# orybkin/video-gcp

Measured on AMD Instinct MI355X. Metric: predicted frames/sec, 64x64x3 seq_len=80 gcp_tree (posterior forward + all loss terms, model(inputs) and model.loss() of train.py:157-159, batch-stat BatchNorm), higher is better.
Workload: dtype f32 (encoder / decoder convs and the tree GEMMs from 512 rows: split-f16 MFMA with f32 accumulate, f32-equivalent; everything else exact f32 MFMA)

## Files before the change

### video-gcp_amd/csrc/gemm.hip

```cpp
#include "common.h"
#include "gemm_tile.h"

#include <cstdio>
#include <cstdlib>
#include <type_traits>

bool gcpx_gemm_split_applies(const gcpx_gemm_args* a);
int gcpx_launch_gemm_split(const gcpx_gemm_args* a, hipStream_t stream);
bool gcpx_gemm_planes_applies(const gcpx_gemm_args* a);
int gcpx_launch_gemm_planes(const gcpx_gemm_args* a, hipStream_t stream);

namespace {

template <int PR, int CR, bool LSTM, bool KS = false>
__global__ void __launch_bounds__(256) gemm_kernel(const gcpx_gemm_args a) {
    gemm_tile<PR, CR, LSTM, KS>(a, blockIdx.x, blockIdx.y, blockIdx.z);
}

__global__ void __launch_bounds__(256) gemm_group_kernel(const gcpx_gemm_args* __restrict__ tab, const int4* __restrict__ dims, const int n) {
    int p = 0;
    while (p + 1 < n && (int)blockIdx.x >= dims[p + 1].x) ++p;
    const int4 d = dims[p];
    const int local = blockIdx.x - d.x;
    const int bx = local % d.y, by = (local / d.y) % d.z, bz = local / (d.y * d.z);
    const gcpx_gemm_args& a = tab[p];
    if (a.epi == GCPX_EPI_GAUSS_SAMPLE) {
        const int r = bx * 16 + ((int)threadIdx.x >> 4), d = by * 16 + ((int)threadIdx.x & 15);
        if (r < a.M) {
            const int b = r / a.rpb, j = r % a.rpb;
            const float* m = a.src[0].ptr + (size_t)b * a.src[0].sb + (size_t)j * a.src[0].sr;
            const float e = a.src[1].ptr[(size_t)b * a.src[1].sb + (size_t)j * a.src[1].sr + d];
            a.out[(size_t)b * a.ob + (size_t)j * a.orow + d] = m[d] + expf(m[a.N + d]) * e;
        }
        return;
    }
    if (a.epi == GCPX_EPI_LSTM) gemm_tile<1, 1, true, true>(a, bx, by, bz);
    else gemm_tile<1, 1, false, true>(a, bx, by, bz);
}

struct TileChoice { int pr, cr; };

TileChoice choose_tile(int M, int N, int nb = 1) {
    if (const char* ov = getenv("GCPX_GEMM_TILE")) {
        int pr = 0, cr = 0, mm = 0;
        if (sscanf(ov, "%d,%d,%d", &pr, &cr, &mm) == 3 && M >= mm && N % (16 * cr) == 0) return TileChoice{pr, cr};
    }
    static const long simds = [] {
        int dev = 0, cus = 256;
        if (hipGetDevice(&dev) == hipSuccess) (void)hipDeviceGetAttribute(&cus, hipDeviceAttributeMultiprocessorCount, dev);
        return 4L * (cus > 0 ? cus : 256);
    }();
    const int prs[3] = {4, 2, 1}, crs[3] = {4, 2, 1};
    TileChoice best{1, 1};
    double best_cost = -1.0, best_bytes = 0.0;
    const long NT = N / 16, RT = (M + 15) / 16;
    if (M >= 64 && N % 64 == 0 && ((RT + 3) / 4) * (NT / 4) * nb >= simds) return TileChoice{4, 4};
    for (int pi = 0; pi < 3; ++pi)
        for (int ci = 0; ci < 3; ++ci) {
            const int pr = prs[pi], cr = crs[ci];
            if (N % (16 * cr)) continue;
            if (pr > 1 && 16 * pr > ((M + 15) & ~15)) continue;
            const long waves = ((RT + pr - 1) / pr) * ((NT + cr - 1) / cr) * nb;
            const long rounds = (waves + simds - 1) / simds;
            const int area = pr * cr;
            const double e = area >= 16 ? 4.2 : area >= 8 ? 4.9 : area >= 4 ? 5.0 : area >= 2 ? 6.0 : 8.0;
            const double compute = (double)rounds * area * e * (rounds > 1 ? 1.35 : 1.0);
            const double bytes = 256.0 * (pr + cr) / area;
            const double l2 = (double)RT * NT * nb * 256.0 * bytes / 1.0e7;
            const double cost = compute > l2 ? compute : l2;
            if (best_cost < 0 || cost < best_cost - 1e-9 || (cost < best_cost + 1e-9 && bytes < best_bytes)) {
                best_cost = cost; best_bytes = bytes; best = TileChoice{pr, cr};
            }
        }
    return best;
}

template <int PR, int CR>
void launch_t(const gcpx_gemm_args* a, hipStream_t stream) {
    const int rbk = (a->M + 16 * PR - 1) / (16 * PR);
    const int cbk = (a->N / 16 + 4 * CR - 1) / (4 * CR);
    const int nb = a->nbatch > 1 ? a->nbatch : 1;
    if (a->epi == GCPX_EPI_LSTM)
        hipLaunchKernelGGL((gemm_kernel<PR, CR, true>), dim3(rbk, cbk, nb), dim3(256), 0, stream, *a);
    else
        hipLaunchKernelGGL((gemm_kernel<PR, CR, false>), dim3(rbk, cbk, nb), dim3(256), 0, stream, *a);
}

}

extern "C" int gcpx_gemm_row_blocks(int32_t M, int32_t N) {
    const TileChoice t = choose_tile(M, N);
    return (M + 16 * t.pr - 1) / (16 * t.pr);
}

static int gemm_check(const gcpx_gemm_args* a);

static bool ks_block_choice(const gcpx_gemm_args* a, int* pr_out, int* cr_out) {
    static const int max_rows = [] { const char* e = getenv("GCPX_GEMM_KS_MAX_ROWS"); return e ? atoi(e) : 4096; }();
    static const int max_cost = [] { const char* e = getenv("GCPX_GEMM_KS_MAX_COST"); return e ? atoi(e) : 6; }();
    if (!(a->M >= 64 && a->M <= max_rows && a->K >= 256 && !a->stats_partial) || getenv("GCPX_GEMM_NO_KS_BLOCKS")) return false;
    static const long cus = [] {
        int dev = 0, n = 256;
        if (hipGetDevice(&dev) == hipSuccess) (void)hipDeviceGetAttribute(&n, hipDeviceAttributeMultiprocessorCount, dev);
        return (long)(n > 0 ? n : 256);
    }();
    const long nb = a->nbatch > 1 ? a->nbatch : 1;
    const int shapes[5][2] = {{1, 1}, {1, 2}, {2, 2}, {4, 2}, {2, 4}};
    int best = 0;
    long best_cost = -1;
    for (int i = 0; i < 5; ++i) {
        const int pr = shapes[i][0], cr = shapes[i][1];
        if (a->N % (16 * cr)) continue;
        const long wgs = (long)((a->M + 16 * pr - 1) / (16 * pr)) * (a->N / (16 * cr)) * nb;
        const long cost = ((wgs + cus - 1) / cus) * (pr + cr);
        if (best_cost < 0 || cost < best_cost) { best_cost = cost; best = i; }
    }
    if (best == 0 || best_cost > max_cost) return false;
    *pr_out = shapes[best][0];
    *cr_out = shapes[best][1];
    return true;
}

static bool gemm_is_small(const gcpx_gemm_args* a) {
    int pr_ = 1, cr_ = 1;
    if (ks_block_choice(a, &pr_, &cr_)) return false;
    const int nb = a->nbatch > 1 ? a->nbatch : 1;
    const TileChoice t = choose_tile(a->M, a->N, nb);
    const long rbk = (a->M + 15) / 16, nt = a->N / 16;
    return t.pr == 1 && t.cr == 1 && a->K >= 256 && rbk * nt * nb <= 1024 && !a->stats_partial;
}

extern "C" int gcpx_gemm_group_dims(const gcpx_gemm_args* host_table, int32_t n, int32_t* dims, int32_t* total_blocks) {
    GCPX_CHECK_ARG(host_table && dims && total_blocks && n >= 1 && n <= 16, "bad arguments");
    int start = 0;
    for (int p = 0; p < n; ++p) {
        if (host_table[p].epi == GCPX_EPI_GAUSS_SAMPLE) {
            const gcpx_gemm_args& a = host_table[p];
            GCPX_CHECK_ARG(a.nsrc == 2 && a.src[0].ptr && a.src[1].ptr && a.out && a.M > 0 && a.N > 0 && a.N % 16 == 0 && a.rpb > 0 &&
                               a.src[0].width == 2 * a.N && a.src[1].width == a.N, "gauss sample: [mu | log_sigma] rows, eps rows, out");
            dims[4 * p] = start; dims[4 * p + 1] = (a.M + 15) / 16; dims[4 * p + 2] = a.N / 16; dims[4 * p + 3] = 1;
            start += dims[4 * p + 1] * dims[4 * p + 2];
            continue;
        }
        const int st = gemm_check(host_table + p);
        if (st != GCPX_OK) return st;
        if (!gemm_is_small(host_table + p)) {
            gcpx_set_error("gcpx_gemm_group_dims: problem %d (M=%d N=%d K=%d) is not in the small-M split-K regime", p, host_table[p].M,
                           host_table[p].N, host_table[p].K);
            return GCPX_ERR_UNSUPPORTED;
        }
        const int nb = host_table[p].nbatch > 1 ? host_table[p].nbatch : 1;
        const int rbk = (host_table[p].M + 15) / 16, nt = host_table[p].N / 16;
        dims[4 * p] = start; dims[4 * p + 1] = rbk; dims[4 * p + 2] = nt; dims[4 * p + 3] = nb;
        start += rbk * nt * nb;
    }
    *total_blocks = start;
    return GCPX_OK;
}

extern "C" int gcpx_gemm_group(const gcpx_gemm_args* dev_table, const int32_t* dev_dims, int32_t n, int32_t total_blocks, void* stream_) {
    hipStream_t stream = reinterpret_cast<hipStream_t>(stream_);
    GCPX_CHECK_ARG(dev_table && dev_dims && n >= 1 && n <= 16 && total_blocks > 0, "bad arguments");
    GCPX_CHECK_ARG((((uintptr_t)dev_dims) & 15) == 0, "dims must be 16-byte aligned");
    hipLaunchKernelGGL(gemm_group_kernel, dim3(total_blocks), dim3(256), 0, stream, dev_table, reinterpret_cast<const int4*>(dev_dims), n);
    GCPX_CHECK_LAUNCH();
    return GCPX_OK;
}

static int gemm_check(const gcpx_gemm_args* a) {
    GCPX_CHECK_ARG(a != nullptr, "null args");
    GCPX_CHECK_ARG(a->epi != GCPX_EPI_GAUSS_SAMPLE, "GCPX_EPI_GAUSS_SAMPLE is a gcpx_gemm_group problem");
    GCPX_CHECK_ARG(a->nsrc >= 1 && a->nsrc <= 6, "nsrc out of range");
    GCPX_CHECK_ARG(a->M > 0 && a->N > 0 && a->N % 16 == 0 && a->rpb > 0, "bad M/N/rpb");
    int ksum = 0;
    for (int s = 0; s < a->nsrc; ++s) {
        GCPX_CHECK_ARG(a->src[s].ptr != nullptr, "source pointer is NULL");
        GCPX_CHECK_ARG(a->src[s].width > 0 && a->src[s].width % 16 == 0, "source width must be a multiple of 16");
        GCPX_CHECK_ARG(!(a->src[s].scale || a->src[s].act) ||
                           (a->src[s].cmod > 0 && (a->src[s].cmod & (a->src[s].cmod - 1)) == 0),
                       "cmod must be a power of two when scale/act is set");
        ksum += a->src[s].width;
    }
    GCPX_CHECK_ARG(ksum == a->K, "K != sum of source widths");
    GCPX_CHECK_ARG(a->wpk != nullptr, "weights missing");
    if (a->epi == GCPX_EPI_LSTM) {
        GCPX_CHECK_ARG(a->c_prev && a->h_out && a->c_out, "LSTM epilogue needs c_prev/h_out/c_out");
    } else {
        GCPX_CHECK_ARG(a->out != nullptr, "out is NULL");
    }
    GCPX_CHECK_ARG(a->nbatch <= 1 || (a->epi != GCPX_EPI_LSTM && !a->stats_partial), "nbatch > 1 only for plain epilogues");
    GCPX_CHECK_ARG(!a->lstm_bwd || (a->epi == GCPX_EPI_NONE && a->nbatch <= 1 && !a->stats_partial),
                   "lstm_bwd: plain epilogue, single problem");
    return GCPX_OK;
}

bool gcpx_gemm_tile_plan(const gcpx_gemm_args* a, int* pr, int* cr, int* ks, int* gx, int* gy, int* gz) {
    if (gemm_check(a) != GCPX_OK || a->stats_partial) return false;
    const int nb = a->nbatch > 1 ? a->nbatch : 1;
    *gz = nb;
    if (ks_block_choice(a, pr, cr)) {
        *ks = 1; *gx = (a->M + 16 * *pr - 1) / (16 * *pr); *gy = a->N / (16 * *cr);
        return true;
    }
    if (gcpx_gemm_split_applies(a)) return false;
    const TileChoice t = choose_tile(a->M, a->N, nb);
    const long rbk = (a->M + 15) / 16, nt = a->N / 16;
    if (t.pr == 1 && t.cr == 1 && a->K >= 256 && !getenv("GCPX_GEMM_NOKS") && rbk * nt * nb <= 1024) {
        *pr = 1; *cr = 1; *ks = 1; *gx = (int)rbk; *gy = (int)nt;
        return true;
    }
    *pr = t.pr; *cr = t.cr; *ks = 0;
    *gx = (a->M + 16 * t.pr - 1) / (16 * t.pr); *gy = (a->N / 16 + 4 * t.cr - 1) / (4 * t.cr);
    return true;
}

extern "C" int gcpx_gemm(const gcpx_gemm_args* a, void* stream_) {
    hipStream_t stream = reinterpret_cast<hipStream_t>(stream_);
    const int st = gemm_check(a);
    if (st != GCPX_OK) return st;
    {
        int pr_ = 1, cr_ = 1;
        if (!ks_block_choice(a, &pr_, &cr_)) {
            if (gcpx_gemm_planes_applies(a)) return gcpx_launch_gemm_planes(a, stream);
            if (gcpx_gemm_split_applies(a)) return gcpx_launch_gemm_split(a, stream);
        }
    }
    const TileChoice t = choose_tile(a->M, a->N, a->nbatch > 1 ? a->nbatch : 1);
    {
        int pr = 1, cr = 1;
        if (ks_block_choice(a, &pr, &cr)) {
            const long nb = a->nbatch > 1 ? a->nbatch : 1;
            const dim3 grid((a->M + 16 * pr - 1) / (16 * pr), a->N / (16 * cr), nb);
            const bool lstm = a->epi == GCPX_EPI_LSTM;
#define GCPX_KS_LAUNCH(PR_, CR_)                                                                                              \
            do {                                                                                                              \
                if (lstm) hipLaunchKernelGGL((gemm_kernel<PR_, CR_, true, true>), grid, dim3(256), 0, stream, *a);            \
                else hipLaunchKernelGGL((gemm_kernel<PR_, CR_, false, true>), grid, dim3(256), 0, stream, *a);                \
            } while (0)
            if (pr == 1 && cr == 2) GCPX_KS_LAUNCH(1, 2);
            else if (pr == 2 && cr == 2) GCPX_KS_LAUNCH(2, 2);
            else if (pr == 4 && cr == 2) GCPX_KS_LAUNCH(4, 2);
            else GCPX_KS_LAUNCH(2, 4);
#undef GCPX_KS_LAUNCH
            GCPX_CHECK_LAUNCH();
            return GCPX_OK;
        }
    }
    if (t.pr == 1 && t.cr == 1 && a->K >= 256 && !getenv("GCPX_GEMM_NOKS")) {
        const long nb = a->nbatch > 1 ? a->nbatch : 1;
        const long rbk = (a->M + 15) / 16, nt = a->N / 16;
        if (rbk * nt * nb <= 1024) {
            if (a->epi == GCPX_EPI_LSTM)
                hipLaunchKernelGGL((gemm_kernel<1, 1, true, true>), dim3(rbk, nt, nb), dim3(256), 0, stream, *a);
            else
                hipLaunchKernelGGL((gemm_kernel<1, 1, false, true>), dim3(rbk, nt, nb), dim3(256), 0, stream, *a);
            GCPX_CHECK_LAUNCH();
            return GCPX_OK;
        }
    }
    switch (t.pr * 10 + t.cr) {
        case 44: launch_t<4, 4>(a, stream); break;
        case 42: launch_t<4, 2>(a, stream); break;
        case 41: launch_t<4, 1>(a, stream); break;
        case 24: launch_t<2, 4>(a, stream); break;
        case 22: launch_t<2, 2>(a, stream); break;
        case 21: launch_t<2, 1>(a, stream); break;
        case 14: launch_t<1, 4>(a, stream); break;
        case 12: launch_t<1, 2>(a, stream); break;
        default: launch_t<1, 1>(a, stream); break;
    }
    GCPX_CHECK_LAUNCH();
    return GCPX_OK;
}
```

### video-gcp_amd/csrc/gemm_split.hip

```cpp
#include "common.h"

#include <cstdlib>
#include <type_traits>

namespace {

typedef _Float16 h8 __attribute__((ext_vector_type(8)));
typedef _Float16 h4 __attribute__((ext_vector_type(4)));
typedef const f32x4 __attribute__((address_space(1)))* gptr4;
__device__ __forceinline__ float4 gload4(const float* p) {
    const f32x4 t = *(gptr4)p;
    return make_float4(t[0], t[1], t[2], t[3]);
}

__device__ __forceinline__ f32x4 mfma32h(h8 a, h8 b, f32x4 c) {
    return __builtin_amdgcn_mfma_f32_16x16x32_f16(a, b, c, 0, 0, 0);
}

template <int TN, int NSUB, int NW = 4>
struct GsCfg {
    static constexpr int TM = 16 * NW, THREADS = 64 * NW, KS = 32 * NSUB;
    static constexpr int NCT = TN / 16;
    static constexpr int W_SUB = NCT * 2048;
    static constexpr int W_BYTES = NSUB * W_SUB;
    static constexpr int X_SUB = NW * 2048;
    static constexpr int X_BYTES = NSUB * X_SUB;
    static constexpr int STAGE = W_BYTES + X_BYTES + 4 * TM;
    static constexpr int LDS_BYTES = 2 * STAGE;
    static constexpr int WLD = W_BYTES / (THREADS * 16);
    static constexpr int WSTEP = THREADS * 16;
};

template <int TN, int NSUB, bool LSTM, bool XF, int NW = 4>
__global__ void __launch_bounds__(64 * NW) gemm_split_kernel(const gcpx_gemm_args a) {
    using Cfg = GsCfg<TN, NSUB, NW>;
    constexpr int KS = Cfg::KS;
    constexpr int NCT = Cfg::NCT, WLD = Cfg::WLD, CPW = NCT / 2;
    extern __shared__ float4 smem4[];
    char* smem = reinterpret_cast<char*>(smem4);
    const int tid = threadIdx.x, lane = tid & 63, wave = tid >> 6;
    const int j = lane & 15, q = lane >> 4;
    const int wr = wave >> 1, wc = wave & 1;
    const int zb = blockIdx.z;
    const int NT = a.N / 16;
    const int ct0 = blockIdx.y * NCT;
    const int M = a.M, rpb = a.rpb;
    const int NK = a.K / KS;

    const int srow = (wave << 4) + j, kq = q;
    const int sr_ = blockIdx.x * Cfg::TM + srow;
    const bool srv = sr_ < M;
    const int srs = srv ? sr_ : 0;
    const int srb = srs / rpb, srj = srs % rpb;
    const int ew = a.w_split_log2_dev ? a.w_split_log2_dev[zb] : a.w_split_log2;
    const int ex_cap = min(100, 126 - ew);
    int ex_run = ex_cap;
    int cur_s = -1, krem = 0, kloc = 0;
    const float* xp = nullptr;
    float xmask = 0.f;
    const float* sp[6];
    float sm[6];
    int sw[6];
#pragma unroll
    for (int i = 0; i < 6; ++i) {
        sp[i] = a.src[0].ptr; sm[i] = 0.f; sw[i] = 0;
        if (i < a.nsrc) {
            sw[i] = a.src[i].width / KS;
            const gcpx_row_src& src = a.src[i];
            bool ok = srv;
            size_t off;
            if (src.rowidx) {
                off = (size_t)src.rowidx[srs] * src.sr;
            } else {
                const int jj = srj + src.shift;
                ok = ok && jj >= 0 && jj < rpb;
                off = (size_t)srb * src.sb + (size_t)(ok ? jj : 0) * src.sr;
            }
            sp[i] = src.ptr + (size_t)zb * a.z_src_off + off + kq * 8;
            sm[i] = ok ? 1.f : 0.f;
        }
    }
    auto next_source = [&]() {
        ++cur_s;
        xp = sp[0]; xmask = sm[0]; krem = sw[0];
#pragma unroll
        for (int i = 1; i < 6; ++i)
            if (cur_s == i) { xp = sp[i]; xmask = sm[i]; krem = sw[i]; }
        kloc = 0;
    };
    const char* wsrc = reinterpret_cast<const char*>(a.wpk_split) + (size_t)zb * a.z_w_off * 4 + (size_t)ct0 * 2048 + tid * 16;

    struct RegSet {
        float4 x[2 * NSUB], w[WLD];
        float mask;
        int src, k0;
    };
    RegSet rs[2];
    const float* last_x = sp[0];
    int last_s = 0;
    auto issue = [&](const int s, RegSet& r) __attribute__((always_inline)) {
        if (s < NK) {
            if (krem == 0) next_source();
            last_x = xp + kloc;
            last_s = s;
            r.mask = xmask; r.src = cur_s; r.k0 = kloc;
            kloc += KS;
            --krem;
        }
#pragma unroll
        for (int h = 0; h < NSUB; ++h) {
            r.x[2 * h] = gload4(last_x + 32 * h);
            r.x[2 * h + 1] = gload4(last_x + 32 * h + 4);
        }
#pragma unroll
        for (int i = 0; i < WLD; ++i) {
            const int sub = i / (WLD / NSUB), c = i % (WLD / NSUB);
            r.w[i] = *reinterpret_cast<const float4*>(wsrc + ((size_t)(NSUB * last_s + sub) * NT) * 2048 + c * Cfg::WSTEP);
        }
    };
    auto commit = [&](const int st, RegSet& r) __attribute__((always_inline)) {
        char* base = smem + st * Cfg::STAGE;
#pragma unroll
        for (int i = 0; i < WLD; ++i) {
            const int sub = i / (WLD / NSUB), c = i % (WLD / NSUB);
            *reinterpret_cast<float4*>(base + sub * Cfg::W_SUB + c * Cfg::WSTEP + tid * 16) = r.w[i];
        }
        if constexpr (XF) {
#pragma unroll
            for (int si = 0; si < 6; ++si) {
                if (r.src == si && (a.src[si].scale || a.src[si].act)) {
#pragma unroll
                    for (int i = 0; i < 2 * NSUB; ++i)
                        r.x[i] = affine_act4(r.x[i], a.src[si].scale, a.src[si].shiftv,
                                             (r.k0 + 32 * (i >> 1) + 4 * (i & 1) + kq * 8) & (a.src[si].cmod - 1), a.src[si].act);
                }
            }
        }
        float amax = 0.f;
#pragma unroll
        for (int i = 0; i < 2 * NSUB; ++i) {
            float4 v = r.x[i];
            v.x *= r.mask; v.y *= r.mask; v.z *= r.mask; v.w *= r.mask;
            r.x[i] = v;
            amax = fmaxf(amax, fmaxf(fmaxf(fabsf(v.x), fabsf(v.y)), fmaxf(fabsf(v.z), fabsf(v.w))));
        }
        {
            unsigned u = __float_as_uint(amax);
            auto s16 = __builtin_amdgcn_permlane16_swap(u, u, false, false);
            u = max(s16[0], s16[1]);
            auto s32 = __builtin_amdgcn_permlane32_swap(u, u, false, false);
            amax = __uint_as_float(max(s32[0], s32[1]));
        }
        if (amax > 0.f) {
            const int ec = 14 + 127 - (int)((__float_as_uint(amax) >> 23) & 0xff);
            ex_run = min(ex_run, max(-100, ec));
        }
        const float sc = __uint_as_float((unsigned)(127 + ex_run) << 23);
        char* xb = base + Cfg::W_BYTES + (wave * 2) * 1024 + lane * 16;
#pragma unroll
        for (int h = 0; h < NSUB; ++h) {
            const float4 v0 = r.x[2 * h], v1 = r.x[2 * h + 1];
            const float f[8] = {v0.x * sc, v0.y * sc, v0.z * sc, v0.w * sc, v1.x * sc, v1.y * sc, v1.z * sc, v1.w * sc};
            h8 p1, p2;
#pragma unroll
            for (int e = 0; e < 8; ++e) {
                p1[e] = (_Float16)f[e];
                p2[e] = (_Float16)fmaf((float)p1[e], -1.f, f[e]);
            }
            *reinterpret_cast<h8*>(xb + h * Cfg::X_SUB) = p1;
            *reinterpret_cast<h8*>(xb + h * Cfg::X_SUB + 1024) = p2;
        }
        if (kq == 0) *reinterpret_cast<int*>(base + Cfg::W_BYTES + Cfg::X_BYTES + srow * 4) = ex_run;
    };

    f32x4 acc[CPW][2];
#pragma unroll
    for (int c = 0; c < CPW; ++c) { acc[c][0] = f32x4{0, 0, 0, 0}; acc[c][1] = f32x4{0, 0, 0, 0}; }
    int excur[2] = {ex_cap, ex_cap};
    auto compute = [&](const int st) __attribute__((always_inline)) {
        const char* base = smem + st * Cfg::STAGE;
        int en[2];
#pragma unroll
        for (int i = 0; i < 2; ++i) en[i] = *reinterpret_cast<const int*>(base + Cfg::W_BYTES + Cfg::X_BYTES + ((2 * wr + i) * 16 + j) * 4);
        if (__any(en[0] != excur[0] || en[1] != excur[1])) {
#pragma unroll
            for (int i = 0; i < 2; ++i) {
                const int d = en[i] - excur[i];
                const float r = d < -126 ? 0.f : __uint_as_float((unsigned)(127 + d) << 23);
#pragma unroll
                for (int c = 0; c < CPW; ++c) acc[c][i] *= r;
                excur[i] = en[i];
            }
        }
#pragma unroll
        for (int sub = 0; sub < NSUB; ++sub) {
            h8 b[2][2];
#pragma unroll
            for (int i = 0; i < 2; ++i) {
                const char* bp = base + Cfg::W_BYTES + sub * Cfg::X_SUB + ((2 * wr + i) * 2) * 1024 + lane * 16;
                b[i][0] = *reinterpret_cast<const h8*>(bp);
                b[i][1] = *reinterpret_cast<const h8*>(bp + 1024);
            }
            constexpr int CH = CPW <= 4 ? CPW : 2;
#pragma unroll
            for (int c0 = 0; c0 < CPW; c0 += CH) {
                h8 w[CH][2];
#pragma unroll
                for (int c = 0; c < CH; ++c) {
                    const char* wp = base + sub * Cfg::W_SUB + ((wc * CPW + c0 + c) * 2) * 1024 + lane * 16;
                    w[c][0] = *reinterpret_cast<const h8*>(wp);
                    w[c][1] = *reinterpret_cast<const h8*>(wp + 1024);
                }
#pragma unroll
                for (int c = 0; c < CH; ++c)
#pragma unroll
                    for (int i = 0; i < 2; ++i) acc[c0 + c][i] = mfma32h(w[c][1], b[i][0], acc[c0 + c][i]);
#pragma unroll
                for (int c = 0; c < CH; ++c)
#pragma unroll
                    for (int i = 0; i < 2; ++i) acc[c0 + c][i] = mfma32h(w[c][0], b[i][1], acc[c0 + c][i]);
#pragma unroll
                for (int c = 0; c < CH; ++c)
#pragma unroll
                    for (int i = 0; i < 2; ++i) acc[c0 + c][i] = mfma32h(w[c][0], b[i][0], acc[c0 + c][i]);
            }
        }
    };

    issue(0, rs[0]);
    issue(1, rs[1]);
    commit(0, rs[0]);
    issue(2, rs[0]);
    __syncthreads();
    for (int s = 0; s < NK; s += 2) {
        compute(0);
        __builtin_amdgcn_sched_barrier(0);
        commit(1, rs[1]);
        issue(s + 3, rs[1]);
        __syncthreads();
        if (s + 1 >= NK) break;
        compute(1);
        __builtin_amdgcn_sched_barrier(0);
        commit(0, rs[0]);
        issue(s + 4, rs[0]);
        __syncthreads();
    }

#pragma unroll
    for (int i = 0; i < 2; ++i) {
        const int r = blockIdx.x * Cfg::TM + (2 * wr + i) * 16 + j;
        const bool rv = r < M;
        const int rs = rv ? r : 0;
        const int rb = rs / rpb, rj = rs % rpb;
        const float inv = __uint_as_float((unsigned)(127 - excur[i] - ew) << 23);
#pragma unroll
        for (int c = 0; c < CPW; ++c) {
            const int nt = ct0 + wc * CPW + c;
            const int n = nt * 16 + q * 4;
            float4 bv = make_float4(0.f, 0.f, 0.f, 0.f);
            if (a.bias) bv = *reinterpret_cast<const float4*>(a.bias + (size_t)zb * a.z_bias_off + n);
            f32x4 v = acc[c][i];
            v[0] = fmaf(v[0], inv, bv.x); v[1] = fmaf(v[1], inv, bv.y); v[2] = fmaf(v[2], inv, bv.z); v[3] = fmaf(v[3], inv, bv.w);
            if (!rv) continue;
            if constexpr (LSTM) {
                const int u = nt * 4 + q;
                const float cp = a.c_prev[(size_t)r * a.c_prev_stride + u];
                const float ig = sigmoidf_(v[0]), fg = sigmoidf_(v[1]), gg = tanhf(v[2]), og = sigmoidf_(v[3]);
                const float cn = fg * cp + ig * gg;
                const float h = og * tanhf(cn);
                const size_t o = (size_t)rb * a.hb + (size_t)rj * a.hrow + u;
                a.h_out[o] = h;
                a.c_out[o] = cn;
                if (a.h_copy) a.h_copy[(size_t)r * (a.N / 4) + u] = h;
                if (a.gates_out)
                    *reinterpret_cast<float4*>(a.gates_out + ((size_t)r * (a.N / 4) + u) * 4) = make_float4(ig, fg, gg, og);
            } else {
                if (a.epi == GCPX_EPI_LRELU) {
                    v[0] = lrelu(v[0], 0.2f); v[1] = lrelu(v[1], 0.2f); v[2] = lrelu(v[2], 0.2f); v[3] = lrelu(v[3], 0.2f);
                }
                float* op = a.out + (size_t)zb * a.z_out_off + (size_t)rb * a.ob + (size_t)rj * a.orow + n;
                *reinterpret_cast<float4*>(op) = make_float4(v[0], v[1], v[2], v[3]);
            }
        }
    }
}

template <int TN, int NSUB, int NW = 4>
int launch_split(const gcpx_gemm_args* a, hipStream_t stream) {
    using Cfg = GsCfg<TN, NSUB, NW>;
    static bool attr_set = false;
    if (!attr_set) {
        for (const void* k : {reinterpret_cast<const void*>(gemm_split_kernel<TN, NSUB, false, false, NW>), reinterpret_cast<const void*>(gemm_split_kernel<TN, NSUB, true, false, NW>),
                              reinterpret_cast<const void*>(gemm_split_kernel<TN, NSUB, false, true, NW>), reinterpret_cast<const void*>(gemm_split_kernel<TN, NSUB, true, true, NW>)}) {
            hipError_t e = hipFuncSetAttribute(k, hipFuncAttributeMaxDynamicSharedMemorySize, Cfg::LDS_BYTES);
            if (e != hipSuccess) {
                gcpx_set_error("gemm split: hipFuncSetAttribute(%d B LDS): %s", Cfg::LDS_BYTES, hipGetErrorString(e));
                return GCPX_ERR_HIP;
            }
        }
        attr_set = true;
    }
    const int nb = a->nbatch > 1 ? a->nbatch : 1;
    const dim3 grid((a->M + Cfg::TM - 1) / Cfg::TM, a->N / TN, nb);
    bool xf = false;
    for (int s = 0; s < a->nsrc; ++s) xf = xf || a->src[s].scale || a->src[s].act;
    const bool lstm = a->epi == GCPX_EPI_LSTM;
    auto kern = lstm ? (xf ? gemm_split_kernel<TN, NSUB, true, true, NW> : gemm_split_kernel<TN, NSUB, true, false, NW>)
                     : (xf ? gemm_split_kernel<TN, NSUB, false, true, NW> : gemm_split_kernel<TN, NSUB, false, false, NW>);
    hipLaunchKernelGGL(kern, grid, dim3(Cfg::THREADS), Cfg::LDS_BYTES, stream, *a);
    GCPX_CHECK_LAUNCH();
    return GCPX_OK;
}

}

bool gcpx_gemm_split_applies(const gcpx_gemm_args* a) {
    static const int min_rows = [] { const char* e = getenv("GCPX_GEMM_SPLIT_MIN_ROWS"); return e ? atoi(e) : 512; }();
    if (!a->wpk_split || a->M < min_rows || a->N % 64 || a->stats_partial || a->lstm_bwd) return false;
    for (int s = 0; s < a->nsrc; ++s)
        if (a->src[s].width % 64) return false;
    return true;
}

int gcpx_launch_gemm_split(const gcpx_gemm_args* a, hipStream_t stream) {
    const long nb = a->nbatch > 1 ? a->nbatch : 1;
    const long rbk = (a->M + 63) / 64;
    static const int force = [] { const char* e = getenv("GCPX_GEMM_SPLIT_CFG"); return e ? atoi(e) : 0; }();
    if (force == 1282) return launch_split<128, 2>(a, stream);
    if (force == 642) return launch_split<64, 2>(a, stream);
    if (force == 641) return launch_split<64, 1>(a, stream);
    if (force == 1281) return launch_split<128, 1>(a, stream);
    if (force == 2561 && a->N % 256 == 0) return launch_split<256, 1>(a, stream);
    if (force == 1288 && a->N % 128 == 0) return launch_split<128, 1, 8>(a, stream);
    if (force == 2568 && a->N % 256 == 0) return launch_split<256, 1, 8>(a, stream);
    if (a->N % 256 == 0 && ((a->M + 127) / 128) * (long)(a->N / 256) * nb >= 256) return launch_split<256, 1, 8>(a, stream);
    if (a->N % 128 == 0 && ((a->M + 127) / 128) * (long)(a->N / 128) * nb >= 512) return launch_split<128, 1, 8>(a, stream);
    if (a->N % 128 == 0 && rbk * (a->N / 128) * nb >= 768) return launch_split<128, 1>(a, stream);
    return launch_split<64, 1>(a, stream);
}
```

### video-gcp_amd/csrc/mlp.hip

```cpp
#include "common.h"
#include "gemm_tile.h"

#include <cstdlib>

bool gcpx_gemm_tile_plan(const gcpx_gemm_args* a, int* pr, int* cr, int* ks, int* gx, int* gy, int* gz);

namespace {

template <int MID, bool LEAN>
__device__ __forceinline__ void mlp_rows(const gcpx_mlp_args& a, const int bx, const int by, const int ny, float* hid) {
    constexpr int NTM = MID / 16;
    constexpr int NW = NTM >= 4 ? 4 : NTM;
    constexpr int TPW = NTM / NW;
    constexpr int PITCH = MID + 4;
    constexpr int CPG = MID / 8;
    static_assert(CPG == 4 || CPG == 16, "GroupNorm group must be one lane (4) or one 16-channel tile");

    const int lane = threadIdx.x & 63, wave = threadIdx.x >> 6;
    const int j = lane & 15, q = lane >> 4;
    const int r = bx * 16 + j;
    const bool rv = r < a.M;
    const int rs = rv ? r : 0;
    const int rb = rs / a.rpb, rj = rs % a.rpb;
    const float slope = a.lrelu_slope;
    const bool owner = wave < NW;
    const int nt0 = wave * TPW;

    f32x4 acc[TPW];
#pragma unroll
    for (int t = 0; t < TPW; ++t) acc[t] = f32x4{0, 0, 0, 0};

    auto load_hidden = [&](const int l, float4 (&w)[NTM][TPW]) {
        const float4* wbase = reinterpret_cast<const float4*>(a.w_mid) + ((size_t)l * NTM * NTM + nt0) * 64 + lane;
#pragma unroll
        for (int kg = 0; kg < NTM; ++kg)
#pragma unroll
            for (int t = 0; t < TPW; ++t) w[kg][t] = wbase[(kg * NTM + t) * 64];
    };
    float4 wA[NTM][TPW], wB[NTM][TPW];
    if (!LEAN && owner && a.n_mid > 0) load_hidden(0, wA);

    if (owner) {
        const float4* wbase = reinterpret_cast<const float4*>(a.w_in) + (size_t)nt0 * 64 + lane;
        int kg0 = 0;
        for (int s = 0; s < a.nsrc; ++s) {
            const gcpx_row_src src = a.src[s];
            bool ok = rv;
            size_t off;
            if (src.rowidx) {
                off = (size_t)src.rowidx[rs] * src.sr;
            } else {
                const int jj = rj + src.shift;
                ok = ok && jj >= 0 && jj < a.rpb;
                off = (size_t)rb * src.sb + (size_t)(ok ? jj : 0) * src.sr;
            }
            const float* bp = src.ptr + off + q * 4;
            const float mask = ok ? 1.f : 0.f;
            const int nkg = src.width / 16;
            const bool xf = src.scale || src.act;
            constexpr int UKI = LEAN ? 4 : 8;
            auto load_set = [&](const int kg, float4 (&b)[UKI], float4 (&w)[UKI][TPW]) {
#pragma unroll
                for (int u = 0; u < UKI; ++u) {
                    const int k = (kg + u < nkg) ? kg + u : nkg - 1;
                    b[u] = *reinterpret_cast<const float4*>(bp + k * 16);
#pragma unroll
                    for (int t = 0; t < TPW; ++t) w[u][t] = wbase[((size_t)(kg0 + k) * NTM + t) * 64];
                }
            };
            auto mfma_set = [&](const int kg, float4 (&b)[UKI], float4 (&w)[UKI][TPW]) {
#pragma unroll
                for (int u = 0; u < UKI; ++u) {
                    if (kg + u < nkg) {
                        float4 bb = b[u];
                        if (xf) bb = affine_act4(bb, src.scale, src.shiftv, ((kg + u) * 16 + q * 4) & (src.cmod - 1), src.act);
                        bb.x *= mask; bb.y *= mask; bb.z *= mask; bb.w *= mask;
#pragma unroll
                        for (int t = 0; t < TPW; ++t) {
                            acc[t] = mfma16(w[u][t].x, bb.x, acc[t]);
                            acc[t] = mfma16(w[u][t].y, bb.y, acc[t]);
                            acc[t] = mfma16(w[u][t].z, bb.z, acc[t]);
                            acc[t] = mfma16(w[u][t].w, bb.w, acc[t]);
                        }
                    }
                }
            };
            float4 b0[UKI], w0[UKI][TPW], b1[UKI], w1[UKI][TPW];
            int kg = 0;
            load_set(0, b0, w0);
            while (true) {
                const int kn = kg + UKI;
                if (kn < nkg) load_set(kn, b1, w1);
                mfma_set(kg, b0, w0);
                if (kn >= nkg) break;
                kg = kn + UKI;
                if (kg < nkg) load_set(kg, b0, w0);
                mfma_set(kn, b1, w1);
                if (kg >= nkg) break;
            }
            kg0 += nkg;
        }
#pragma unroll
        for (int t = 0; t < TPW; ++t) {
            const int c = (nt0 + t) * 16 + q * 4;
            const float4 bv = *reinterpret_cast<const float4*>(a.b_in + c);
            float4 v = make_float4(lrelu(acc[t][0] + bv.x, slope), lrelu(acc[t][1] + bv.y, slope),
                                   lrelu(acc[t][2] + bv.z, slope), lrelu(acc[t][3] + bv.w, slope));
            *reinterpret_cast<float4*>(hid + j * PITCH + c) = v;
            if (a.save && rv && by == 0) *reinterpret_cast<float4*>(a.save + (size_t)r * MID + c) = v;
        }
    }
    __syncthreads();

    int cur = 0;
    auto hidden = [&](const int l, float4 (&w)[NTM][TPW], float4 (&wnext)[NTM][TPW]) {
        const float* hin = hid + cur * 16 * PITCH;
        float* hout = hid + (cur ^ 1) * 16 * PITCH;
        if (owner) {
            float4 b[NTM];
#pragma unroll
            for (int kg = 0; kg < NTM; ++kg) b[kg] = *reinterpret_cast<const float4*>(hin + j * PITCH + kg * 16 + q * 4);
            if constexpr (LEAN) load_hidden(l, w);
            else if (l + 1 < a.n_mid) load_hidden(l + 1, wnext);
#pragma unroll
            for (int t = 0; t < TPW; ++t) acc[t] = f32x4{0, 0, 0, 0};
#pragma unroll
            for (int kg = 0; kg < NTM; ++kg) {
#pragma unroll
                for (int t = 0; t < TPW; ++t) {
                    acc[t] = mfma16(w[kg][t].x, b[kg].x, acc[t]);
                    acc[t] = mfma16(w[kg][t].y, b[kg].y, acc[t]);
                    acc[t] = mfma16(w[kg][t].z, b[kg].z, acc[t]);
                    acc[t] = mfma16(w[kg][t].w, b[kg].w, acc[t]);
                }
            }
#pragma unroll
            for (int t = 0; t < TPW; ++t) {
                const int c = (nt0 + t) * 16 + q * 4;
                const float4 bv = *reinterpret_cast<const float4*>(a.b_mid + l * MID + c);
                const float4 gv = *reinterpret_cast<const float4*>(a.gn_gamma + l * MID + c);
                const float4 be = *reinterpret_cast<const float4*>(a.gn_beta + l * MID + c);
                const float v0 = acc[t][0] + bv.x, v1 = acc[t][1] + bv.y, v2 = acc[t][2] + bv.z, v3 = acc[t][3] + bv.w;
                float sum = (v0 + v1) + (v2 + v3);
                if (CPG == 16) { sum += __shfl_xor(sum, 16); sum += __shfl_xor(sum, 32); }
                const float mean = sum * (1.f / CPG);
                const float d0 = v0 - mean, d1 = v1 - mean, d2 = v2 - mean, d3 = v3 - mean;
                float ss = (d0 * d0 + d1 * d1) + (d2 * d2 + d3 * d3);
                if (CPG == 16) { ss += __shfl_xor(ss, 16); ss += __shfl_xor(ss, 32); }
                const float rstd = rsqrtf(ss * (1.f / CPG) + a.gn_eps);
                float4 o = make_float4(lrelu(d0 * rstd * gv.x + be.x, slope), lrelu(d1 * rstd * gv.y + be.y, slope),
                                       lrelu(d2 * rstd * gv.z + be.z, slope), lrelu(d3 * rstd * gv.w + be.w, slope));
                *reinterpret_cast<float4*>(hout + j * PITCH + c) = o;
                if (a.save && rv && by == 0) {
                    float* sv = a.save + (size_t)(1 + 2 * l) * a.M * MID + (size_t)r * MID + c;
                    *reinterpret_cast<float4*>(sv) = make_float4(v0, v1, v2, v3);
                    *reinterpret_cast<float4*>(sv + (size_t)a.M * MID) = o;
                }
            }
        }
        cur ^= 1;
        __syncthreads();
    };
    if constexpr (LEAN) {
        for (int l = 0; l < a.n_mid; ++l) hidden(l, wA, wA);
    } else {
        for (int l = 0; l < a.n_mid; l += 2) {
            hidden(l, wA, wB);
            if (l + 1 < a.n_mid) hidden(l + 1, wB, wA);
        }
    }

    const float* hin = hid + cur * 16 * PITCH;
    float4 b[NTM];
#pragma unroll
    for (int kg = 0; kg < NTM; ++kg) b[kg] = *reinterpret_cast<const float4*>(hin + j * PITCH + kg * 16 + q * 4);
    const int out_pad = (a.out_dim + 15) & ~15;
    const int NTO = out_pad / 16;
    const float4* wbase = reinterpret_cast<const float4*>(a.w_out) + lane;
    const int split = a.out_split > 0 ? a.out_split : a.out_dim;
    float* orow = a.out ? a.out + (size_t)rb * a.ob + (size_t)rj * a.orow : nullptr;
    const int tstart = by * 4 + wave, tstride = ny * 4;

    if (a.epi == GCPX_MLP_GAUSS) {
        const int nz = a.out_dim / 2;
        const int NTZ = nz / 16;
        const float* erow = a.eps + (size_t)rb * a.eb + (size_t)rj * a.erow;
        float* zrow = a.z + (size_t)rb * a.zb + (size_t)rj * a.zrow;
        for (int nt = tstart; nt < NTZ; nt += tstride) {
            float4 wm[NTM], wl[NTM];
#pragma unroll
            for (int kg = 0; kg < NTM; ++kg) {
                wm[kg] = wbase[(kg * NTO + nt) * 64];
                wl[kg] = wbase[(kg * NTO + nt + NTZ) * 64];
            }
            f32x4 am = f32x4{0, 0, 0, 0}, al = f32x4{0, 0, 0, 0};
#pragma unroll
            for (int kg = 0; kg < NTM; ++kg) {
                am = mfma16(wm[kg].x, b[kg].x, am); al = mfma16(wl[kg].x, b[kg].x, al);
                am = mfma16(wm[kg].y, b[kg].y, am); al = mfma16(wl[kg].y, b[kg].y, al);
                am = mfma16(wm[kg].z, b[kg].z, am); al = mfma16(wl[kg].z, b[kg].z, al);
                am = mfma16(wm[kg].w, b[kg].w, am); al = mfma16(wl[kg].w, b[kg].w, al);
            }
            if (rv) {
                const int n = nt * 16 + q * 4;
                const float4 bm = *reinterpret_cast<const float4*>(a.b_out + n);
                const float4 bl = *reinterpret_cast<const float4*>(a.b_out + nz + n);
                const float4 mu = make_float4(am[0] + bm.x, am[1] + bm.y, am[2] + bm.z, am[3] + bm.w);
                const float4 ls = make_float4(al[0] + bl.x, al[1] + bl.y, al[2] + bl.z, al[3] + bl.w);
                if (orow) {
                    *reinterpret_cast<float4*>(orow + n) = mu;
                    *reinterpret_cast<float4*>(orow + nz + n) = ls;
                }
                const float4 e = *reinterpret_cast<const float4*>(erow + n);
                float4 z;
                z.x = mu.x + expf(ls.x) * e.x; z.y = mu.y + expf(ls.y) * e.y;
                z.z = mu.z + expf(ls.z) * e.z; z.w = mu.w + expf(ls.w) * e.w;
                *reinterpret_cast<float4*>(zrow + n) = z;
            }
        }
    } else {
        for (int nt = tstart; nt < NTO; nt += tstride) {
            float4 w[NTM];
#pragma unroll
            for (int kg = 0; kg < NTM; ++kg) w[kg] = wbase[(kg * NTO + nt) * 64];
            f32x4 ao = f32x4{0, 0, 0, 0};
#pragma unroll
            for (int kg = 0; kg < NTM; ++kg) {
                ao = mfma16(w[kg].x, b[kg].x, ao);
                ao = mfma16(w[kg].y, b[kg].y, ao);
                ao = mfma16(w[kg].z, b[kg].z, ao);
                ao = mfma16(w[kg].w, b[kg].w, ao);
            }
            if (rv) {
                const int n = nt * 16 + q * 4;
                if (n < a.out_dim) {
                    const float4 bv = *reinterpret_cast<const float4*>(a.b_out + n);
                    float v[4] = {ao[0] + bv.x, ao[1] + bv.y, ao[2] + bv.z, ao[3] + bv.w};
                    if (a.epi == GCPX_MLP_TANH) { v[0] = tanhf(v[0]); v[1] = tanhf(v[1]); v[2] = tanhf(v[2]); v[3] = tanhf(v[3]); }
                    const int blk = n / split, nn = n % split;
                    float* op = orow + (size_t)blk * a.oblk + nn;
                    if (n + 3 < a.out_dim && nn + 3 < split && (((uintptr_t)op) & 15) == 0) {
                        *reinterpret_cast<float4*>(op) = make_float4(v[0], v[1], v[2], v[3]);
                    } else {
#pragma unroll
                        for (int k = 0; k < 4; ++k) {
                            const int nk = n + k;
                            if (nk < a.out_dim) orow[(size_t)(nk / split) * a.oblk + nk % split] = v[k];
                        }
                    }
                }
            }
        }
    }
}

__device__ __forceinline__ void prefetch_range(const float* base, const size_t n_floats, const int slot, const int nslots) {
    const size_t n4 = n_floats / 4;
    const float4* p = reinterpret_cast<const float4*>(base);
    for (size_t i = (size_t)slot * 256 + threadIdx.x; i < n4; i += (size_t)nslots * 256) {
        const float4 v = p[i];
        asm volatile("" ::"v"(v.x), "v"(v.y), "v"(v.z), "v"(v.w));
    }
}

__device__ __forceinline__ void prefetch_weights(const gcpx_mlp_args& a, const int helper, const int nhelpers) {
    const int nslots = nhelpers >= 8 ? nhelpers / 8 : 1;
    const int slot = nhelpers >= 8 ? helper / 8 : helper;
    if (slot >= nslots) return;
    const int out_pad = (a.out_dim + 15) & ~15;
    prefetch_range(a.w_in, (size_t)a.in_dim * a.mid, slot, nslots);
    if (a.n_mid) prefetch_range(a.w_mid, (size_t)a.n_mid * a.mid * a.mid, slot, nslots);
    prefetch_range(a.w_out, (size_t)a.mid * out_pad, slot, nslots);
}

template <int MID, bool LEAN>
__global__ void __launch_bounds__(256, LEAN ? 2 : 1) mlp_kernel(const gcpx_mlp_args a, const int nblocks) {
    __shared__ float4 hid4[2 * 16 * (MID + 4) / 4];
    const int gx = (a.M + 15) / 16;
    if ((int)blockIdx.x >= nblocks) {
        prefetch_weights(a, blockIdx.x - nblocks, gridDim.x - nblocks);
        return;
    }
    mlp_rows<MID, LEAN>(a, blockIdx.x % gx, blockIdx.x / gx, nblocks / gx, reinterpret_cast<float*>(hid4));
}

template <int MID, bool LEAN>
__global__ void __launch_bounds__(256, LEAN ? 2 : 1) mlp_group_kernel(const gcpx_mlp_args* __restrict__ tab, const int4* __restrict__ dims, const int n,
                                                                      const int nblocks) {
    __shared__ float4 hid4[2 * 16 * (MID + 4) / 4];
    if ((int)blockIdx.x >= nblocks) {
        for (int p = 0; p < n; ++p) prefetch_weights(tab[p], blockIdx.x - nblocks, gridDim.x - nblocks);
        return;
    }
    int p = 0;
    while (p + 1 < n && (int)blockIdx.x >= dims[p + 1].x) ++p;
    const int4 d = dims[p];
    const int local = blockIdx.x - d.x;
    mlp_rows<MID, LEAN>(tab[p], local % d.y, local / d.y, d.z, reinterpret_cast<float*>(hid4));
}

template <int MID, int PR, int CR, bool KS>
__global__ void __launch_bounds__(256, 1) level_pre_kernel(const gcpx_mlp_args* __restrict__ tab, const int4* __restrict__ dims, const int n,
                                                           const int nblocks, const gcpx_gemm_args g, const int gx, const int gy, const int gz) {
    __shared__ float4 hid4[2 * 16 * (MID + 4) / 4];
    const int blk = blockIdx.x;
    if (blk >= nblocks) {
        const int local = blk - nblocks, ng = gx * gy * gz;
        if (local < ng) {
            gemm_tile<PR, CR, false, KS>(g, local % gx, (local / gx) % gy, local / (gx * gy));
        } else {
            for (int p = 0; p < n; ++p) prefetch_weights(tab[p], local - ng, gridDim.x - nblocks - ng);
        }
        return;
    }
    int p = 0;
    while (p + 1 < n && blk >= dims[p + 1].x) ++p;
    const int4 d = dims[p];
    const int local = blk - d.x;
    mlp_rows<MID, false>(tab[p], local % d.y, local / d.y, d.z, reinterpret_cast<float*>(hid4));
}

typedef void (*level_pre_fn)(const gcpx_mlp_args*, const int4*, int, int, const gcpx_gemm_args, int, int, int);
level_pre_fn level_pre_variant(const int pr, const int cr, const int ks) {
    if (ks) {
        if (pr == 1 && cr == 1) return level_pre_kernel<128, 1, 1, true>;
        if (pr == 1 && cr == 2) return level_pre_kernel<128, 1, 2, true>;
        if (pr == 2 && cr == 2) return level_pre_kernel<128, 2, 2, true>;
        if (pr == 4 && cr == 2) return level_pre_kernel<128, 4, 2, true>;
        if (pr == 2 && cr == 4) return level_pre_kernel<128, 2, 4, true>;
        return nullptr;
    }
    if (pr == 2 && cr == 2) return level_pre_kernel<128, 2, 2, false>;
    if (pr == 4 && cr == 2) return level_pre_kernel<128, 4, 2, false>;
    return nullptr;
}

int mlp_check(const gcpx_mlp_args* a) {
    GCPX_CHECK_ARG(a != nullptr, "null args");
    GCPX_CHECK_ARG(a->nsrc >= 1 && a->nsrc <= 6, "nsrc out of range");
    GCPX_CHECK_ARG(a->M > 0 && a->rpb > 0, "bad M/rpb");
    int ksum = 0;
    for (int s = 0; s < a->nsrc; ++s) {
        GCPX_CHECK_ARG(a->src[s].ptr != nullptr, "source pointer is NULL");
        GCPX_CHECK_ARG(a->src[s].width > 0 && a->src[s].width % 16 == 0, "source width must be a multiple of 16");
        ksum += a->src[s].width;
    }
    GCPX_CHECK_ARG(ksum == a->in_dim, "in_dim != sum of source widths");
    GCPX_CHECK_ARG(a->w_in && a->b_in && a->w_out && a->b_out, "weights missing");
    GCPX_CHECK_ARG(a->n_mid == 0 || (a->w_mid && a->b_mid && a->gn_gamma && a->gn_beta), "hidden-layer weights missing");
    if (a->epi == GCPX_MLP_GAUSS) {
        GCPX_CHECK_ARG(a->out_dim % 32 == 0 && a->eps && a->z, "GAUSS epilogue needs out_dim % 32 == 0, eps, z");
    } else {
        GCPX_CHECK_ARG(a->out != nullptr, "out is NULL");
    }
    return GCPX_OK;
}

void mlp_grid(const gcpx_mlp_args* a, int* gx, int* gy) {
    *gx = (a->M + 15) / 16;
    const int head_tiles = ((a->epi == GCPX_MLP_GAUSS ? a->out_dim / 2 : a->out_dim) + 15) / 16;
    static const int ymax = [] { const char* e = getenv("GCPX_MLP_GY_MAX"); return e ? atoi(e) : 32; }();
    int y = 1;
    while (y < ymax && *gx * y < 256 && head_tiles / (4 * y) >= 2) y *= 2;
    *gy = y;
}

int mlp_helpers(const int nb, const int cus) {
    static const int cap = [] { const char* e = getenv("GCPX_MLP_HELPERS"); return e ? atoi(e) : 1 << 30; }();
    if (nb > cus / 4) return 0;
    const int h = ((cus - nb) / 8) * 8;
    return h < cap ? (h > 0 ? h : 0) : cap;
}

}

extern "C" int gcpx_mlp_group_dims(const gcpx_mlp_args* host_table, int32_t n, int32_t* dims, int32_t* total_blocks) {
    GCPX_CHECK_ARG(host_table && dims && total_blocks && n >= 1 && n <= 16, "bad arguments");
    int start = 0;
    for (int p = 0; p < n; ++p) {
        const int st = mlp_check(host_table + p);
        if (st != GCPX_OK) return st;
        GCPX_CHECK_ARG(host_table[p].mid == host_table[0].mid, "all problems of a group share the hidden width");
        int gx, gy;
        mlp_grid(host_table + p, &gx, &gy);
        dims[4 * p] = start; dims[4 * p + 1] = gx; dims[4 * p + 2] = gy; dims[4 * p + 3] = 0;
        start += gx * gy;
    }
    *total_blocks = start;
    return GCPX_OK;
}

extern "C" int gcpx_mlp_group(const gcpx_mlp_args* dev_table, const int32_t* dev_dims, int32_t n, int32_t total_blocks, int32_t mid,
                              void* stream_) {
    hipStream_t stream = reinterpret_cast<hipStream_t>(stream_);
    GCPX_CHECK_ARG(dev_table && dev_dims && n >= 1 && n <= 16 && total_blocks > 0, "bad arguments");
    GCPX_CHECK_ARG((((uintptr_t)dev_dims) & 15) == 0, "dims must be 16-byte aligned");
    const int cus = gcpx_conv_grid() / 2;
    const bool lean = total_blocks > cus;
    const int grid = total_blocks + mlp_helpers(total_blocks, cus);
    const int4* dd = reinterpret_cast<const int4*>(dev_dims);
    if (mid == 128 && lean) hipLaunchKernelGGL((mlp_group_kernel<128, true>), dim3(grid), dim3(256), 0, stream, dev_table, dd, n, total_blocks);
    else if (mid == 128) hipLaunchKernelGGL((mlp_group_kernel<128, false>), dim3(grid), dim3(256), 0, stream, dev_table, dd, n, total_blocks);
    else if (mid == 32 && lean) hipLaunchKernelGGL((mlp_group_kernel<32, true>), dim3(grid), dim3(256), 0, stream, dev_table, dd, n, total_blocks);
    else if (mid == 32) hipLaunchKernelGGL((mlp_group_kernel<32, false>), dim3(grid), dim3(256), 0, stream, dev_table, dd, n, total_blocks);
    else {
        gcpx_set_error("gcpx_mlp_group: unsupported mid=%d (128 or 32)", mid);
        return GCPX_ERR_UNSUPPORTED;
    }
    GCPX_CHECK_LAUNCH();
    return GCPX_OK;
}

extern "C" int gcpx_mlp_group_gemm_supported(const gcpx_gemm_args* g, int32_t total_blocks, int32_t mid) {
    if (!g || mid != 128 || g->epi == GCPX_EPI_LSTM || g->epi == GCPX_EPI_GAUSS_SAMPLE) return 0;
    const int cus = gcpx_conv_grid() / 2;
    if (total_blocks > cus) return 0;
    int pr, cr, ks, gx, gy, gz;
    if (!gcpx_gemm_tile_plan(g, &pr, &cr, &ks, &gx, &gy, &gz)) return 0;
    return level_pre_variant(pr, cr, ks) != nullptr;
}

extern "C" int gcpx_mlp_group_gemm(const gcpx_mlp_args* dev_table, const int32_t* dev_dims, int32_t n, int32_t total_blocks, int32_t mid,
                                   const gcpx_gemm_args* g, void* stream_) {
    hipStream_t stream = reinterpret_cast<hipStream_t>(stream_);
    GCPX_CHECK_ARG(dev_table && dev_dims && g && n >= 1 && n <= 16 && total_blocks > 0, "bad arguments");
    GCPX_CHECK_ARG((((uintptr_t)dev_dims) & 15) == 0, "dims must be 16-byte aligned");
    int pr, cr, ks, gx, gy, gz;
    level_pre_fn kern = nullptr;
    if (mid == 128 && g->epi != GCPX_EPI_LSTM && g->epi != GCPX_EPI_GAUSS_SAMPLE && gcpx_gemm_tile_plan(g, &pr, &cr, &ks, &gx, &gy, &gz))
        kern = level_pre_variant(pr, cr, ks);
    if (!kern) {
        gcpx_set_error("gcpx_mlp_group_gemm: this GEMM / hidden width has no combined launch (ask gcpx_mlp_group_gemm_supported)");
        return GCPX_ERR_UNSUPPORTED;
    }
    const int cus = gcpx_conv_grid() / 2;
    const int work = total_blocks + gx * gy * gz;
    const int grid = work + mlp_helpers(work, cus);
    hipLaunchKernelGGL(kern, dim3(grid), dim3(256), 0, stream, dev_table, reinterpret_cast<const int4*>(dev_dims), n, total_blocks, *g, gx, gy, gz);
    GCPX_CHECK_LAUNCH();
    return GCPX_OK;
}

extern "C" int gcpx_mlp(const gcpx_mlp_args* a, void* stream_) {
    hipStream_t stream = reinterpret_cast<hipStream_t>(stream_);
    const int st = mlp_check(a);
    if (st != GCPX_OK) return st;
    int gx, gy;
    mlp_grid(a, &gx, &gy);
    const int cus = gcpx_conv_grid() / 2;
    const bool lean = gx * gy > cus;
    const int nb = gx * gy, grid = nb + mlp_helpers(nb, cus);
    if (a->mid == 128 && lean) hipLaunchKernelGGL((mlp_kernel<128, true>), dim3(grid), dim3(256), 0, stream, *a, nb);
    else if (a->mid == 128) hipLaunchKernelGGL((mlp_kernel<128, false>), dim3(grid), dim3(256), 0, stream, *a, nb);
    else if (a->mid == 32 && lean) hipLaunchKernelGGL((mlp_kernel<32, true>), dim3(grid), dim3(256), 0, stream, *a, nb);
    else if (a->mid == 32) hipLaunchKernelGGL((mlp_kernel<32, false>), dim3(grid), dim3(256), 0, stream, *a, nb);
    else {
        gcpx_set_error("gcpx_mlp: unsupported mid=%d (128 or 32)", a->mid);
        return GCPX_ERR_UNSUPPORTED;
    }
    GCPX_CHECK_LAUNCH();
    return GCPX_OK;
}
```

### video-gcp_amd/forward_plan.py

```python
import ctypes as C
import os
from contextlib import contextmanager

import torch

from . import packing as pk
from . import runtime as rt
from .hparams import GCPHParams
from .params import init_params, encoder_layers, encoder_skip_layers, decoder_layers
from .plan_ops import _Plan, _addr, N_LANES


class ForwardPlanMixin:

    def _plan_encoder(self, plan, tag, x_ptr, F, out_ptr, out_ob, out_orow, out_rpb):
        hp, P, lib = self._hp, self.pk, self.lib
        G = lib.gcpx_conv4x4s2_grid()
        S = hp.img_sz
        skip_idx = encoder_skip_layers(hp)
        skips = {}
        a0 = self._buf(f"{tag}.a0", (F, S // 2, S // 2, hp.ngf))
        enc_rec = dict(F=F, x_ptr=x_ptr, a0=a0, r={}, out=(out_ptr, out_ob, out_orow, out_rpb))
        plan.rec[f"enc:{tag}"] = enc_rec
        plan.add(f"enc.input:{tag}", lib.gcpx_conv4x4s2_image, x_ptr, P["enc.input.w"].data_ptr(),
                 P["enc.input.b"].data_ptr(), a0.data_ptr(), F, S, S, hp.ngf, rt.ACT_LRELU)
        prev = (a0.data_ptr(), hp.ngf, 1, None, None, rt.ACT_NONE)
        if 0 in skip_idx:
            skips[0] = (a0, hp.ngf, None, None, rt.ACT_NONE)
        res = S // 2
        for li, (name, cin, cout, norm) in enumerate(self._enc_layers[1:], start=1):
            r = self._buf(f"{tag}.r{li}", (F, res // 2, res // 2, cout))
            enc_rec["r"][li] = r
            stats = self._buf(f"{tag}.st{li}", (G, 2, cout)) if self.training else None
            a = self._conv_args([prev], F, res, res, res // 2, res // 2, cout, cout, P[f"enc.{name}.w"],
                                P[f"enc.{name}.b"], r, stats=stats)
            self._set_split(a, f"enc.{name}")
            plan.keep.append(a)
            plan.add(f"enc.{name}:{tag}", lib.gcpx_conv4x4s2, C.byref(a))
            res //= 2
            scale, shift = self._bn(plan, f"{tag}.bn{li}", f"encoder.net.{name}.norm", cout, stats, G, cout,
                                    F * res * res)
            prev = (r.data_ptr(), cout, 1, scale, shift, rt.ACT_LRELU)
            if li in skip_idx:
                skips[li] = (r, cout, scale, shift, rt.ACT_LRELU)
        assert res == 4
        ctop = self._c_top
        src = self._rowsrc(prev[0], 16 * ctop, 16 * ctop, 16 * ctop, scale=prev[3], shiftv=prev[4], act=prev[5], cmod=ctop)
        src.sb, src.sr = out_rpb * 16 * ctop, 16 * ctop
        self._gemm(plan, f"enc.head:{tag}", [src], F, hp.nz_enc, out_rpb, P["enc.head.w"], P["enc.head.b"],
                   out=out_ptr, ob=out_ob, orow=out_orow)
        return skips

    def _plan_seq_encoder(self, plan, tag, prefix, enc_traj, out, B):
        hp, P, lib = self._hp, self.pk, self.lib
        T, nz = hp.max_seq_len, hp.nz_enc
        y1 = self._buf(f"{tag}.y1", (B * T, hp.nz_mid))
        y2 = self._buf(f"{tag}.y2", (B * T, hp.nz_mid))
        taps = lambda t, w, **kw: [self._rowsrc(t.data_ptr(), T * w, w, w, shift=d, **kw) for d in (-1, 0, 1)]
        self._gemm(plan, f"{tag}.input", taps(enc_traj, nz), B * T, hp.nz_mid, T, P[f"{tag}.input.w"], P[f"{tag}.input.b"],
                   out=y1.data_ptr(), ob=T * hp.nz_mid, orow=hp.nz_mid, epi=rt.EPI_LRELU)
        assert hp.conv_inf_enc_layers == 1
        nrb = lib.gcpx_gemm_row_blocks(B * T, hp.nz_mid)
        st = self._buf(f"{tag}.st", (nrb, 2, hp.nz_mid)) if self.training else None
        self._gemm(plan, f"{tag}.pyramid-0", taps(y1, hp.nz_mid), B * T, hp.nz_mid, T, P[f"{tag}.pyramid-0.w"],
                   P[f"{tag}.pyramid-0.b"], out=y2.data_ptr(), ob=T * hp.nz_mid, orow=hp.nz_mid, stats=st)
        sc, sh = self._bn(plan, f"{tag}.bn", f"{prefix}.net.pyramid-0.norm", hp.nz_mid, st, nrb, hp.nz_mid, B * T)
        self._gemm(plan, f"{tag}.head", taps(y2, hp.nz_mid, scale=sc, shiftv=sh, act=rt.ACT_LRELU, cmod=hp.nz_mid),
                   B * T, nz, T, P[f"{tag}.head.w"], P[f"{tag}.head.b"], out=out.data_ptr(), ob=T * nz, orow=nz)

    def _plan_attention(self, plan, l, W, el, er, M, n, B, Kp, Vp, tin):
        hp, lib = self._hp, self.lib
        T, nz, dk = hp.max_seq_len, hp.nz_enc, hp.nz_attn_key
        li = l if hp.untied_layers else 0
        qin = self._buf(f"attn.qin{l}", (M, dk))
        self._mlp(plan, f"attn.query{l}", W["attn.query"], [el, er], M, n, out=qin.data_ptr(), ob=n * dk, orow=dk)
        dense = lambda t, w: self._rowsrc(t.data_ptr(), 0, w, w)
        qp = self._buf(f"attn.q{l}", (M, dk))
        self._gemm(plan, f"attn.q_proj{l}", [dense(qin, dk)], M, dk, M, W["attn.q_proj.w"], W["attn.q_proj.b"],
                   out=qp.data_ptr(), ob=0, orow=dk)
        o = self._buf(f"attn.o{l}", (M, nz))
        gamma = self._buf(f"attn.gamma{l}", (M, T))
        temp = self.sd[f"tree_module.tree_modules.{li}.inference.attention.attention_layers.0.temperature"]
        plan.add(f"attn{l}", lib.gcpx_attention, qp.data_ptr(), _addr(Kp, li * B * T * dk), _addr(Vp, li * B * T * nz), None,
                 tin["end_ind"].data_ptr(), temp.data_ptr(), o.data_ptr(), gamma.data_ptr(), M, n, T, dk, nz, hp.n_attention_heads)
        raw = self._buf(f"attn.raw{l}", (M, nz))
        self._gemm(plan, f"attn.out_proj{l}", [dense(o, nz)], M, nz, M, W["attn.out_proj.w"], W["attn.out_proj.b"],
                   out=raw.data_ptr(), ob=0, orow=nz)
        et = self._buf(f"attn.e_tilde{l}", (M, nz))
        self._gemm(plan, f"attn.out{l}", [dense(raw, nz)], M, nz, M, W["attn.out.w"], W["attn.out.b"], out=et.data_ptr(), ob=0, orow=nz)
        plan.rec.setdefault("gamma", {})[l] = gamma
        plan.rec.setdefault("e_tilde", {})[l] = et
        plan.rec.setdefault("attn", {})[l] = dict(qin=qin, qp=qp, o=o, raw=raw, gamma=gamma, et=et, M=M, n=n, li=li, temp=temp)
        return self._rowsrc(et.data_ptr(), n * nz, nz, nz)

    def _plan_decoder_features(self, plan, e_src, F, rpb, skips):
        hp, P, lib = self._hp, self.pk, self.lib
        ctop = self._c_top
        d0 = self._buf("dec.d0", (F, 4, 4, ctop))
        plan.rec["dec"] = dict(F=F, rpb=rpb, e_src=e_src, d0=d0, blocks=[], skips=skips)
        nrb = lib.gcpx_gemm_row_blocks(F, 16 * ctop)
        st = self._buf("dec.st0", (nrb, 2, 16 * ctop)) if self.training else None
        self._gemm(plan, "dec.input", [e_src], F, 16 * ctop, rpb, P["dec.input.w"], P["dec.input.b"], out=d0.data_ptr(),
                   ob=rpb * 16 * ctop, orow=16 * ctop, stats=st)
        sc, sh = self._bn(plan, "dec.bn0", "decoder.net.input.norm", ctop, st, nrb, 16 * ctop, F * 16)
        prev = (d0.data_ptr(), ctop, 1, sc, sh, rt.ACT_LRELU)
        res = 4
        for name, c_prev, c_skip, skip_idx, cout in decoder_layers(hp):
            srcs = [prev]
            if skip_idx >= 0:
                t, C_, ssc, ssh, sact = skips[skip_idx]
                assert C_ == c_skip and t.shape[1] == res
                srcs.append((t.data_ptr(), C_, rpb, ssc, ssh, sact))
            o = self._buf(f"dec.{name}", (F, 2 * res, 2 * res, cout))
            cpad = (cout + 15) // 16 * 16
            hoist = (skip_idx >= 0 and rpb > 1 and F % rpb == 0 and self.split_f16 and cout in (32, 64) and c_prev % 32 == 0 and
                     c_skip % 32 == 0 and f"dec.{name}" in self.pk_split and "fold" not in self.pk_split[f"dec.{name}"] and
                     os.environ.get("GCPX_NO_SKIP_HOIST") is None)
            addend = None
            if hoist:
                addend = self._buf(f"dec.{name}.skip", (F // rpb, 2 * res, 2 * res, cout))
                t, C_, ssc, ssh, sact = skips[skip_idx]
                zb = self._buf(f"dec.{name}.zero_bias", (cpad,), zero=True)
                a_s = self._conv_args([(t.data_ptr(), C_, 1, ssc, ssh, sact)], F // rpb, res, res, 2 * res, 2 * res, cout, cout,
                                      P[f"dec.{name}.w"], zb, addend, upsample=1)
                self._set_split(a_s, f"dec.{name}")
                a_s.wpk_split = a_s.wpk_split + (c_prev // 32) * 9 * (cpad // 16) * 2048
                plan.keep.append(a_s)
                plan.add(f"dec.{name}.skip", lib.gcpx_conv3x3, C.byref(a_s))
                srcs_main = [prev]
            else:
                srcs_main = srcs
            a = self._conv_args(srcs_main, F, res, res, 2 * res, 2 * res, cout, cout, P[f"dec.{name}.w"], P[f"dec.{name}.b"],
                                o, upsample=1, stats=(o if self.training else None))
            if hoist:
                a.addend, a.addend_frame_div = addend.data_ptr(), rpb
            self._set_split(a, f"dec.{name}")
            Gl = lib.gcpx_conv3x3_grid(C.byref(a))
            assert Gl > 0, rt.lib().gcpx_last_error()
            st = self._buf(f"dec.st.{name}", (Gl, 2, cpad)) if self.training else None
            a.stats_partial = st.data_ptr() if st is not None else None
            plan.keep.append(a)
            plan.add(f"dec.{name}", lib.gcpx_conv3x3, C.byref(a))
            plan.rec["dec"]["blocks"].append(dict(name=name, srcs=srcs, out=o, res_in=res, cout=cout, c_prev=c_prev, c_skip=c_skip,
                                                  skip_idx=skip_idx))
            res *= 2
            sc, sh = self._bn(plan, f"dec.bn.{name}", f"decoder.net.{name}.norm", cout, st, Gl, cpad, F * res * res)
            prev = (o.data_ptr(), cout, 1, sc, sh, rt.ACT_LRELU)
        assert res == hp.img_sz
        return prev

    def _build_plan(self, key, tin):
        hp, P, lib = self._hp, self.pk, self.lib
        B, has_traj, has_z, sample_prior, phase = key[0], key[1], key[2], key[3], key[4]
        pred_len = key[9]
        train_aux = has_traj and phase == "train" and not sample_prior
        L, T, N = hp.hierarchy_levels, hp.max_seq_len, hp.n_nodes
        nz, nv, H, SD = hp.nz_enc, hp.nz_vae, hp.nz_mid_lstm, hp.lstm_state_dim
        PS = 2 ** L + 1
        plan = _Plan(lib)
        G = lib.gcpx_conv_grid()
        def plan_aux_indices():
            AUXK = ("inv_t0", "inv_t1", "cost_start_idx", "cost_end_idx")
            plan.add("aux_sample_indices", lib.gcpx_aux_sample_indices_gauss, tin["end_ind"].data_ptr(), tin["aux_n"].data_ptr(), B,
                     hp.inv_mdl_temp_dist, *[tin[k].data_ptr() for k in AUXK])
        if "aux_n" in tin and pred_len:
            plan_aux_indices()

        E = self._buf("E", (B, PS, nz))
        Hid = self._buf("Hid", (B, PS, SD))
        Z = self._buf("Z", (B, PS, nv))
        PZ = self._buf("PZ", (B, PS, 2 * nv))
        QZ = self._buf("QZ", (B, PS, 2 * nv))
        node_t = self._buf("node_t", (B, N), torch.int32)
        leave = self._buf("leave", (B, N), torch.int32)
        f2n = self._buf("frame2node", (B, T), torch.int32)
        etrow = self._buf("etilde_row", (B * N,), torch.int32)
        seq_len = self._buf("seq_len", (B,), torch.int32)
        kept_idx = self._buf("kept_idx", (B, T), torch.int32)
        node2row = self._buf("node2row", (B, N), torch.int32)

        adaptive, attentive = hp.adaptive, hp.attentive_inference
        if adaptive:
            kept_idx = self._buf("kept_idx", (B, N), torch.int32)
        def plan_bookkeeping():
            if not adaptive:
                plan.add("balanced_binding", lib.gcpx_balanced_binding, tin["end_ind"].data_ptr(), B, L, T, node_t.data_ptr(),
                         leave.data_ptr(), f2n.data_ptr(), etrow.data_ptr(), seq_len.data_ptr(), node2row.data_ptr())
                plan.add("compact_index", lib.gcpx_compact_index, leave.data_ptr(), B, N, T, kept_idx.data_ptr())
                r2f = self._buf("row2frame", (B * T,), torch.int32)
                if self._head_grad_fused(key) or self._rows_direct(key):
                    plan.add("row2frame", lib.gcpx_index_inverse, node2row.data_ptr(), B * N, r2f.data_ptr(), B * T)
                if self._head_grad_fused(key):
                    S_ = hp.img_sz
                    dMD = self._buf("bw.dMD", (B * T, S_, S_, self._head_pitch))
                    plan.add("zero_unmapped", lib.gcpx_zero_unmapped_rows, dMD.data_ptr(), S_ * S_ * self._head_pitch, r2f.data_ptr(), B * T)

        enc_traj = inf_enc = None
        plan.fork([1, 2])
        traj_first = os.environ.get("GCPX_ENC_ORDER") != "small_first"
        def plan_traj_encoder():
            nonlocal enc_traj, inf_enc
            plan.lane = 0
            if has_traj:
                enc_traj = self._buf("enc_traj", (B * T, nz))
                self._plan_encoder(plan, "traj", tin["traj_seq"].data_ptr(), B * T, enc_traj.data_ptr(), T * nz, nz, T)
                if hp.seq_enc == "none":
                    inf_enc = enc_traj
                else:
                    inf_enc = self._buf("inf_enc_seq", (B * T, nz))
                    self._plan_seq_encoder(plan, "seq", "inf_encoder", enc_traj, inf_enc, B)
                if attentive:
                    dk = hp.nz_attn_key
                    n_mod = L if hp.untied_layers else 1
                    if hp.seq_enc == "none":
                        kenc = enc_traj
                    else:
                        kenc = self._buf("inf_key_enc", (B * T, nz))
                        self._plan_seq_encoder(plan, "kseq", "inf_key_encoder.0", enc_traj, kenc, B)
                    keys = self._buf("inf_enc_key_seq", (B * T, dk))
                    dense = lambda t, w: self._rowsrc(t.data_ptr(), 0, w, w)
                    self._gemm(plan, "kseq.key", [dense(kenc, nz)], B * T, dk, B * T, P["kseq.key.w"], P["kseq.key.b"],
                               out=keys.data_ptr(), ob=0, orow=dk)
                    Kp = self._buf("attn.K", (n_mod, B * T, dk))
                    Vp = self._buf("attn.V", (n_mod, B * T, nz))
                    self._gemm(plan, "attn.k_proj", [dense(keys, dk)], B * T, dk, B * T, P["attn.k_proj.w"], P["attn.k_proj.b"],
                               out=Kp.data_ptr(), ob=0, orow=dk, batch=(n_mod, 0, P["attn.k_proj.w"][0].numel(), dk, B * T * dk))
                    self._gemm(plan, "attn.v_proj", [dense(inf_enc, nz)], B * T, nz, B * T, P["attn.v_proj.w"], P["attn.v_proj.b"],
                               out=Vp.data_ptr(), ob=0, orow=nz, batch=(n_mod, 0, P["attn.v_proj.w"][0].numel(), nz, B * T * nz))
                    plan.rec["attn_kv"] = dict(Kp=Kp, Vp=Vp, keys=keys, kenc=kenc, n_mod=n_mod)

        if traj_first:
            plan_traj_encoder()
        plan.lane = 1
        if "rng_all" in tin:
            plan.add("randn", lib.gcpx_randn, tin["rng_all"].data_ptr(), tin["rng_all"].numel(), self._buf("rng_state", (2,), torch.int64).data_ptr())
            if "aux_n" in tin and not pred_len:
                plan.wait(2, 1)
        skips = self._plan_encoder(plan, "I0", tin["I_0"].data_ptr(), B, _addr(E), PS * nz, 0, 1)
        plan.lane = 2
        if not pred_len:
            if "aux_n" in tin:
                plan_aux_indices()
            plan_bookkeeping()
        if hp.attach_cost_mdl and hp.run_cost_mdl and train_aux and self._has_aux_training:
            gt = self._buf("cost_target", (B,))
            rows = hp.input_nc * hp.img_sz
            plan.add("path_cost", lib.gcpx_path_cost, tin["traj_seq"].data_ptr(), tin["cost_start_idx"].data_ptr(),
                     tin["cost_end_idx"].data_ptr(), B, T, rows, hp.img_sz, self._buf("cost_partial", (B, rows)).data_ptr(), gt.data_ptr())
        self._plan_encoder(plan, "Ig", tin["I_g"].data_ptr(), B, _addr(E, 2 ** L * nz), PS * nz, 0, 1)
        outs = {}
        e0 = lambda: self._rowsrc(_addr(E), PS * nz, 0, nz)
        eg = lambda: self._rowsrc(_addr(E, 2 ** L * nz), PS * nz, 0, nz)
        if hp.regress_length and not pred_len:
            plan.wait(2, 1)
            logits = self._buf("seq_len_logits", (B, T))
            self._mlp(plan, "length_pred", P["length_pred"], [e0(), eg()], B, 1, out=logits.data_ptr(), ob=T, orow=0)
            outs["seq_len_logits"] = logits
        if not traj_first:
            plan_traj_encoder()
        plan.lane = 0
        plan.join([1, 2])

        if hp.regress_length and pred_len:
            logits = self._buf("seq_len_logits", (B, T))
            self._mlp(plan, "length_pred", P["length_pred"], [e0(), eg()], B, 1, out=logits.data_ptr(), ob=T, orow=0)
            outs["seq_len_logits"] = logits
            plan.add("sample_length", lib.gcpx_sample_length, logits.data_ptr(), tin["len_u"].data_ptr(), B, T, 2, tin["end_ind"].data_ptr())
            plan_bookkeeping()

        side_merge = False
        for l in range(L):
            W = P[f"tree{l if hp.untied_layers else 0}"]
            s = 2 ** (L - 1 - l)
            n = 2 ** l
            M = B * n
            nodeoff = lambda w: s * w
            el = lambda: self._rowsrc(_addr(E), PS * nz, 2 * s * nz, nz)
            er = lambda: self._rowsrc(_addr(E, 2 * s * nz), PS * nz, 2 * s * nz, nz)
            pz_out = (_addr(PZ, nodeoff(2 * nv)), PS * 2 * nv, 2 * s * 2 * nv)
            z_map = (_addr(Z, nodeoff(nv)), PS * nv, 2 * s * nv)
            nl = hp.n_lstm_layers
            merged = self._buf(f"merged{l}", (M, 2 * nl * H))

            def plan_merge(lv=l, group=None):
                s_, n_ = 2 ** (L - 1 - lv), 2 ** lv
                Wl = P[f"tree{lv if hp.untied_layers else 0}"]
                mg = self._buf(f"merged{lv}", (B * n_, 2 * nl * H))
                if hp.tree_lstm == "sum":
                    for side, mode in ((0, 0), (2 * s_ * SD, 1)):
                        plan.add(f"merge{lv}.{mode}", lib.gcpx_rows_strided, _addr(mg), n_ * SD, SD, _addr(Hid, side), PS * SD, 2 * s_ * SD,
                                 B, n_, SD, mode)
                    return
                if hp.tree_lstm == "linear":
                    h1 = self._rowsrc(_addr(Hid), PS * SD, 2 * s_ * SD, SD)
                    h2 = self._rowsrc(_addr(Hid, 2 * s_ * SD), PS * SD, 2 * s_ * SD, SD)
                    self._gemm(plan, f"merge{lv}", [h1, h2], B * n_, SD, n_, Wl["proj.w"], Wl["proj.b"], out=_addr(mg), ob=n_ * SD, orow=SD,
                               group=group)
                    return
                h1 = self._rowsrc(_addr(Hid), PS * SD, 2 * s_ * SD, H)
                h2 = self._rowsrc(_addr(Hid, 2 * s_ * SD), PS * SD, 2 * s_ * SD, H)
                self._gemm(plan, f"merge{lv}", [h1, h2], B * n_, H, n_, Wl["proj.w"], Wl["proj.b"], out=_addr(mg),
                           ob=n_ * 2 * nl * H, orow=2 * nl * H, batch=(2 * nl, H, Wl["proj.w"][0].numel(), H, H), group=group)

            merge_with_predictors = not has_z and not sample_prior and hp.tree_lstm not in ("sum", "")
            if has_z:
                g = (_addr(tin["z"], (s - 1) * nv), N * nv, 2 * s * nv) + z_map
                self._mlp(plan, f"prior{l}", W["prior"], [el(), er()], M, n, out=pz_out[0], ob=pz_out[1], orow=pz_out[2], gauss=g)
            elif sample_prior:
                g = (_addr(tin["eps"], (n - 1) * nv), N * nv, nv) + z_map
                self._mlp(plan, f"prior{l}", W["prior"], [el(), er()], M, n, out=pz_out[0], ob=pz_out[1], orow=pz_out[2], gauss=g)
            else:
                pq = []
                self._mlp(plan, f"prior{l}", W["prior"], [el(), er()], M, n, out=pz_out[0], ob=pz_out[1], orow=pz_out[2], group=pq)
                if attentive:
                    et = self._plan_attention(plan, l, W, el(), er(), M, n, B, plan.rec["attn_kv"]["Kp"], plan.rec["attn_kv"]["Vp"], tin)
                else:
                    et = self._rowsrc(inf_enc.data_ptr(), 0, nz, nz, rowidx=etrow[B * (n - 1):])
                g = (_addr(tin["eps"], (n - 1) * nv), N * nv, nv) + z_map
                self._mlp(plan, f"posterior{l}", W["q"], [el(), er(), et], M, n, out=_addr(QZ, nodeoff(2 * nv)),
                          ob=PS * 2 * nv, orow=2 * s * 2 * nv, gauss=g, group=pq)
                mg = []
                if l > 0 and merge_with_predictors and not side_merge:
                    plan_merge(l, group=mg)
                self._mlp_group(plan, f"prior+posterior{l}", pq, gemm=(mg[0] if mg else None))
                if side_merge:
                    plan.join([1])
                    side_merge = False
            zs = lambda: self._rowsrc(z_map[0], z_map[1], z_map[2], nv)
            if not hp.tree_lstm:
                srcs = [el(), er(), zs()] + ([e0(), eg()] if hp.context_every_step else [])
                self._mlp(plan, f"subgoal{l}", W["sg"], srcs, M, n, out=_addr(E, nodeoff(nz)), ob=PS * nz, orow=2 * s * nz, tanh=True)
                continue
            if l == 0:
                if hp.lstm_init == "zero":
                    for slot in (0, 2 ** L):
                        plan.add(f"lstm_init.zero{slot}", lib.gcpx_rows_strided, _addr(Hid, slot * SD), PS * SD, 0, self._zero_row(SD).data_ptr(),
                                 0, 0, B, 1, SD, 0)
                else:
                    self._mlp(plan, "lstm_init", W["init"], [el(), er(), zs()], M, n, out=_addr(Hid), ob=PS * SD, orow=0,
                              oblk=2 ** L * SD, out_split=SD)
                plan_merge()
            x = self._buf(f"x{l}.0", (M, H))
            srcs = [el(), er(), zs()] + ([e0(), eg()] if hp.context_every_step else [])
            fused = "lstm0f.w" in W and not self.save_for_backward
            if not fused:
                self._gemm(plan, f"embed{l}", srcs, M, H, n, W["embed.w"], W["embed.b"], out=x.data_ptr(), ob=n * H, orow=H)
            for i in range(nl):
                xn = self._buf(f"x{l}.{i + 1}", (M, H))
                xs = self._rowsrc(x.data_ptr(), n * H, H, H)
                hs = self._rowsrc(_addr(merged, 2 * i * H), n * 2 * nl * H, 2 * nl * H, H)
                lstm = (_addr(merged, (2 * i + 1) * H), 2 * nl * H, _addr(Hid, nodeoff(SD) + 2 * i * H),
                        _addr(Hid, nodeoff(SD) + (2 * i + 1) * H), PS * SD, 2 * s * SD, xn.data_ptr())
                if i == 0 and fused:
                    self._gemm(plan, f"lstm{l}.0", srcs + [hs], M, 4 * H, n, W["lstm0f.w"], W["lstm0f.b"], epi=rt.EPI_LSTM, lstm=lstm)
                else:
                    self._gemm(plan, f"lstm{l}.{i}", [xs, hs], M, 4 * H, n, W[f"lstm{i}.w"], W[f"lstm{i}.b"],
                               epi=rt.EPI_LSTM, lstm=lstm)
                x = xn
            g = []
            self._gemm(plan, f"out{l}", [self._rowsrc(x.data_ptr(), n * H, H, H)], M, nz, n, W["out.w"], W["out.b"],
                       out=_addr(E, nodeoff(nz)), ob=PS * nz, orow=2 * s * nz, group=g)
            if l + 1 < L and not merge_with_predictors:
                plan_merge(l + 1, group=g)
            self._gemm_group(plan, f"out{l}+merge{l + 1}" if len(g) > 1 else f"out{l}", g)
            if (l + 1 < L and merge_with_predictors and hp.tree_lstm == "split_linear" and B * 2 ** (l + 1) >= self._merge_side_rows):
                plan.fork([1])
                plan.lane = 1
                plan_merge(l + 1)
                plan.lane = 0
                side_merge = True

        F = B * N
        matching = adaptive and has_traj and phase == "train"

        heads = []

        def plan_aux(idx, Wd):
            mes = self._buf("model_enc_seq", (B, Wd, nz))
            plan.add("gather.model_enc_seq", lib.gcpx_gather_rows, E.data_ptr(), idx.data_ptr(), mes.data_ptr(), B, Wd, PS, 1, nz)
            outs["model_enc_seq_padded"] = mes
            if hp.run_state_regressor:
                rs = self._buf("regressed_state", (B, Wd, hp.state_dim))
                self._mlp(plan, "state_regressor", P["state_regressor"], [self._rowsrc(mes.data_ptr(), Wd * nz, nz, nz)],
                          B * Wd, Wd, out=rs.data_ptr(), ob=Wd * hp.state_dim, orow=hp.state_dim, group=heads)
                outs["regressed_state_padded"] = rs
            if hp.attach_inv_mdl and phase == "train" and (sample_prior or hp.train_inv_mdl_full_seq or not has_traj):
                act = self._buf("actions", (B, Wd - 1, hp.n_actions))
                first = enc_traj if has_traj else mes
                s0 = self._rowsrc(first.data_ptr(), (T if has_traj else Wd) * nz, nz, nz)
                s1 = self._rowsrc(_addr(mes, nz), Wd * nz, nz, nz)
                self._mlp(plan, "inv_mdl", P["inv_mdl"], [s0, s1], B * (Wd - 1), Wd - 1, out=act.data_ptr(),
                          ob=(Wd - 1) * hp.n_actions, orow=hp.n_actions, group=heads)
                outs["actions_padded"] = act
            aux_rows = None
            if train_aux and ((hp.attach_inv_mdl and not hp.train_inv_mdl_full_seq) or (hp.attach_cost_mdl and hp.run_cost_mdl)):
                aux_rows = self._buf("aux_rows", (4, B), torch.int32)
                plan.add("aux_index_rows", lib.gcpx_aux_index_rows, tin["inv_t0"].data_ptr(), tin["inv_t1"].data_ptr(),
                         tin["cost_start_idx"].data_ptr(), tin["cost_end_idx"].data_ptr(), B, T, Wd, aux_rows.data_ptr())
                gather = lambda t, i: self._rowsrc(t.data_ptr(), 0, nz, nz, rowidx=aux_rows[i])
            if hp.attach_inv_mdl and train_aux and not hp.train_inv_mdl_full_seq:
                act = self._buf("actions_sampled", (B, hp.n_actions))
                self._mlp(plan, "inv_mdl", P["inv_mdl"], [gather(enc_traj, 0), gather(mes, 1)], B, B, out=act.data_ptr(), ob=0,
                          orow=hp.n_actions, group=heads)
                outs["actions_sampled"] = act
            if hp.attach_cost_mdl and hp.run_cost_mdl and train_aux:
                cost = self._buf("cost_pred", (B, 1))
                self._mlp(plan, "cost_mdl", P["cost_mdl"], [gather(mes, 2), gather(mes, 3)], B, B, out=cost.data_ptr(), ob=0, orow=1,
                          group=heads)
                outs["cost_pred"], outs["cost_target"] = cost, self._buf("cost_target", (B,))

        heads_lane = 0
        if heads_lane:
            plan.fork([1])
        plan.lane = heads_lane
        if adaptive:
            dist = self._buf("distances", (B, N - 1))
            self._mlp(plan, "distance", P["distance"], [self._rowsrc(_addr(E, nz), PS * nz, nz, nz),
                                                        self._rowsrc(_addr(E, 2 * nz), PS * nz, nz, nz)],
                      B * (N - 1), N - 1, out=dist.data_ptr(), ob=N - 1, orow=1)
            pruned_len = self._buf("pruned_len", (B,), torch.int32)
            plan.add("distance_prune", lib.gcpx_distance_prune, dist.data_ptr(), C.c_float(hp.learned_pruning_threshold), None, B, N,
                     leave.data_ptr(), kept_idx.data_ptr(), pruned_len.data_ptr(), None)
            outs["distances"], outs["pruned_len"] = dist, pruned_len
            if not matching:
                plan_aux(kept_idx, N)
                outs["aux_len"] = pruned_len
        else:
            plan_aux(kept_idx, T)
            exist = self._buf("existence", (B, N))
            self._mlp(plan, "existence", P["existence"], [self._rowsrc(_addr(E, nz), PS * nz, nz, nz)], F, N,
                      out=exist.data_ptr(), ob=N, orow=1, group=heads)
            outs["existence"] = exist
        if heads:
            self._mlp_group(plan, "heads", heads)
            heads.clear()
        plan.lane = 0

        def kl_args(kl_b, batch=()):
            return (_addr(QZ, 2 * nv), _addr(PZ, 2 * nv)) + batch + (N, nv, PS * 2 * nv, 2 * nv, C.c_float(hp.free_nats), None, 0, kl_b.data_ptr())

        def loss_args():
            kl_b = self._buf("kl_b", (B,))
            la = rt.LossArgs()
            la.nll_bt, la.pad_mask, la.kl_b = self._buf("nll_bt", (B, T)).data_ptr(), tin["pad_mask"].data_ptr(), kl_b.data_ptr()
            la.len_logits = outs["seq_len_logits"].data_ptr() if "seq_len_logits" in outs else None
            la.end_ind = tin["end_ind"].data_ptr()
            if adaptive:
                la.existence, la.leave = outs["distances"].data_ptr(), outs["distance_target"].data_ptr()
            else:
                la.existence, la.leave = outs["existence"].data_ptr(), leave.data_ptr()
            if "regressed_state_padded" in outs and "traj_seq_states" in tin:
                la.regressed_state, la.state_target = outs["regressed_state_padded"].data_ptr(), tin["traj_seq_states"].data_ptr()
            la.seq_len = seq_len.data_ptr()
            if "actions_sampled" in outs and "actions" in tin:
                la.action_pred, la.action_seq, la.inv_t0 = outs["actions_sampled"].data_ptr(), tin["actions"].data_ptr(), tin["inv_t0"].data_ptr()
                la.n_actions, la.w_action = hp.n_actions, hp.action_rec_weight
            if "cost_pred" in outs:
                la.cost_pred, la.cost_target, la.w_cost = outs["cost_pred"].data_ptr(), outs["cost_target"].data_ptr(), 1.0
            loss_out = self._buf("losses", (16,), zero=True)
            la.out, la.B, la.T, la.N, la.state_dim = loss_out.data_ptr(), B, T, (N - 1 if adaptive else N), hp.state_dim
            la.w_rec, la.w_kl, la.w_len, la.w_exist, la.w_state = hp.dense_img_rec_weight, hp.kl_weight, hp.length_pred_weight, 1.0, 1.0
            if self._kl_w is not None:
                la.w_kl_dev = self._kl_w.data_ptr()
            la.total_div = float(T * hp.input_nc * hp.img_sz * hp.img_sz)
            plan.keep.append(la)
            return la, kl_b

        decode, with_loss = key[8], key[7]
        loss_pre = None
        if with_loss and not adaptive:
            loss_pre = loss_args()
            plan.add("loss.pre", lib.gcpx_loss_pre, C.byref(loss_pre[0]), *kl_args(loss_pre[1]))
        if decode:
            F = B * N
            S = hp.img_sz
            prev = self._plan_decoder_features(plan, self._rowsrc(_addr(E, nz), PS * nz, nz, nz), F, N, skips)
            images = self._buf("images_df", (B, N, hp.input_nc, S, S))
            distr = matched_distr = None
            with_loss = key[7]
            dlm = hp.decoder_distribution == "discrete_logistic_mixture"
            head_out, row_map = None, None
            fused_nll = None
            if dlm:
                mode = rt.HEAD_DLM_MEAN
                if self.materialize_distr or (adaptive and self.save_for_backward and with_loss):
                    mode, distr = rt.HEAD_DLM_BOTH, self._buf("distr_df", (B, N, S, S, self._head_pitch))
                    head_out = distr
                elif self._head_grad_fused(key):
                    mode, row_map = rt.HEAD_DLM_NLL_GRAD, node2row
                    head_out = self._buf("bw.dMD", (B * T, S, S, self._head_pitch))
                    fused_nll = self._buf("nll_partial", ((S // 4) * (S // 16), B * T), zero=True)
                    plan.rec["nll_bwd_fused"] = plan.rec["head_grad_fused"] = True
                elif with_loss and not adaptive and not self.save_for_backward and self._head_nll_fusable():
                    mode, row_map = rt.HEAD_DLM_NLL, node2row
                    fused_nll = self._buf("nll_partial", ((S // 4) * (S // 16), B * T), zero=True)
                elif with_loss and not adaptive:
                    mode, matched_distr = rt.HEAD_DLM_BOTH, self._buf("matched_distr", (B, T, S, S, self._head_pitch))
                    head_out, row_map = matched_distr, node2row
            else:
                mode = rt.HEAD_TANH_NCHW
            a = self._conv_args([prev], F, S, S, S, S, hp.head_channels, self._head_pitch, P["dec.head.w"], P["dec.head.b"],
                                head_out, upsample=0, head_mode=mode, images=images)
            rows_direct = self._rows_direct(key) and (row_map is not None or mode == rt.HEAD_DLM_MEAN)
            rows_images = None
            if rows_direct:
                row_map = node2row
                want_matched = has_traj and phase == "train"
                rows_images = self._buf("rows_images", (2 if want_matched else 1, B, T, hp.input_nc, S, S))
                a.images_rows = rows_images.data_ptr()
                a.images_rows_dup = rows_images[0].numel() if want_matched else 0
            a.raw_row_map = row_map.data_ptr() if row_map is not None else None
            if fused_nll is not None:
                a.nll_target, a.nll_partial, a.nll_rows = tin["traj_seq"].data_ptr(), fused_nll.data_ptr(), B * T
                if mode == rt.HEAD_DLM_NLL_GRAD:
                    a.nll_row_weight = tin["pad_mask"].data_ptr()
                    a.nll_scale = hp.dense_img_rec_weight / (B * float(T * hp.input_nc * S * S))
            self._set_split(a, "dec.head")
            plan.keep.append(a)
            if heads_lane:
                plan.join([1])
            plan.add("dec.head", lib.gcpx_conv3x3, C.byref(a))
            outs["images_df"], outs["distr_df_kernel_order"] = images, distr

            row = hp.input_nc * S * S
            if matching:
                ns = lib.gcpx_cdist_splits(row)
                dsum = self._buf("cdist.dsum", (B, N, T))
                plan.add("cdist", lib.gcpx_cdist, images.data_ptr(), tin["traj_seq"].data_ptr(), B, N, T, row,
                         self._buf("cdist.part", (ns, B, N, T)).data_ptr(), self._buf("cdist.xn", (B * N,)).data_ptr(),
                         self._buf("cdist.yn", (B * T,)).data_ptr(), dsum.data_ptr())
                wdf = self._buf("match_dist_df", (B, N, T))
                temp = self.sd["tree_module.tree_modules.0.binding.temp"]
                plan.add("soft_dtw", lib.gcpx_soft_dtw, dsum.data_ptr(), C.c_float(float(row)), temp.data_ptr(), tin["end_ind"].data_ptr(),
                         B, N, T, self._buf("dtw.acc", (2 * B, N, T), torch.float64).data_ptr(), wdf.data_ptr())
                outs["dtw_acc"] = self._buf("dtw.acc", (2 * B, N, T), torch.float64)
                matched_idx = self._buf("matched_idx", (B, T), torch.int32)
                best_t = self._buf("best_t", (B, N), torch.int32)
                entropy, p_n = self._buf("entropy", (B, N)), self._buf("p_n", (B, N))
                plan.add("match_stats", lib.gcpx_match_stats, wdf.data_ptr(), tin["end_ind"].data_ptr(), B, L, T, f2n.data_ptr(),
                         matched_idx.data_ptr(), best_t.data_ptr(), entropy.data_ptr(), p_n.data_ptr())
                dist_tgt = self._buf("distance_target", (B, N - 1), torch.int32)
                plan.add("distance_target", lib.gcpx_distance_prune, outs["distances"].data_ptr(),
                         C.c_float(hp.learned_pruning_threshold), best_t.data_ptr(), B, N, leave.data_ptr(), kept_idx.data_ptr(),
                         outs["pruned_len"].data_ptr(), dist_tgt.data_ptr())
                plan.add("seq_len", lib.gcpx_seq_index, tin["end_ind"].data_ptr(), B, T, self._buf("seq_idx", (B, T), torch.int32).data_ptr(),
                         seq_len.data_ptr())
                plan_aux(matched_idx, T)
                self._mlp_group(plan, "heads", heads)
                heads.clear()
                ent_sum = self._buf("entropy_sum", (1,))
                plan.add("entropy_sum", lib.gcpx_reduce_partials, entropy.data_ptr(), B * N, 1, 1, ent_sum.data_ptr(), 0)
                outs["entropy_sum"] = ent_sum
                outs.update(cdist_sum=dsum, match_dist_df=wdf, matched_idx=matched_idx, best_t=best_t, entropy_df=entropy, p_n_df=p_n,
                            distance_target=dist_tgt, aux_len=seq_len)
            elif has_traj and phase == "train":
                if rows_images is not None:
                    matched = rows_images[1]
                    plan.add("gather.matched.rest", lib.gcpx_gather_rows_rest, images.data_ptr(), f2n.data_ptr(), matched.data_ptr(), B, T, N,
                             0, row, self._buf("row2frame", (B * T,), torch.int32).data_ptr())
                else:
                    matched = self._buf("matched_images", (B, T, hp.input_nc, S, S))
                    plan.add("gather.matched", lib.gcpx_gather_rows, images.data_ptr(), f2n.data_ptr(), matched.data_ptr(), B, T, N,
                             0, row)
                outs["soft_matched_estimates"] = matched
            Wp = N if adaptive else T
            if rows_images is not None:
                pruned = rows_images[0]
                plan.add("gather.pruned.rest", lib.gcpx_gather_rows_rest, images.data_ptr(), kept_idx.data_ptr(), pruned.data_ptr(), B, Wp, N,
                         0, row, self._buf("row2frame", (B * T,), torch.int32).data_ptr())
            else:
                pruned = self._buf("pruned_images", (B, Wp, hp.input_nc, S, S))
                plan.add("gather.pruned", lib.gcpx_gather_rows, images.data_ptr(), kept_idx.data_ptr(), pruned.data_ptr(), B, Wp, N, 0,
                         row)
            outs["pruned_padded"] = pruned

        if with_loss:
            nll_bt = self._buf("nll_bt", (B, T))
            if adaptive:
                plan.add("loss.averaging_nll", lib.gcpx_averaging_nll, dsum.data_ptr(), wdf.data_ptr(),
                         self.sd["decoder.log_sigma"].data_ptr(), C.c_float(float(row)), B, N, T, nll_bt.data_ptr())
            elif dlm and fused_nll is not None:
                plan.add("loss.nll_reduce", lib.gcpx_reduce_partials, fused_nll.data_ptr(), fused_nll.shape[0], B * T, B * T,
                         nll_bt.data_ptr(), 0)
            elif dlm:
                if matched_distr is None:
                    matched_distr = self._buf("matched_distr", (B, T, S, S, self._head_pitch))
                    plan.add("gather.matched_distr", lib.gcpx_gather_rows, distr.data_ptr(), f2n.data_ptr(),
                             matched_distr.data_ptr(), B, T, N, 0, S * S * self._head_pitch)
                if self.save_for_backward:
                    dMD = self._buf("bw.dMD", (B * T, S, S, self._head_pitch))
                    div = float(T * hp.input_nc * S * S)
                    plan.add("loss.dlm_nll+bwd", lib.gcpx_dlm_nll_bwd, matched_distr.data_ptr(), tin["traj_seq"].data_ptr(),
                             tin["pad_mask"].data_ptr(), C.c_float(hp.dense_img_rec_weight / (B * div)), dMD.data_ptr(),
                             self._buf("bw.dMD.colsum", (B * T, self._head_pitch)).data_ptr(), nll_bt.data_ptr(), B * T, S * S,
                             self._head_pitch, hp.n_mixtures)
                    plan.rec["nll_bwd_fused"] = True
                else:
                    plan.add("loss.dlm_nll", lib.gcpx_dlm_nll, matched_distr.data_ptr(), tin["traj_seq"].data_ptr(),
                             tin["pad_mask"].data_ptr(), nll_bt.data_ptr(), B * T, S * S, self._head_pitch, hp.n_mixtures)
            else:
                plan.add("loss.gauss_nll", lib.gcpx_gauss_nll, outs["soft_matched_estimates"].data_ptr(),
                         tin["traj_seq"].data_ptr(), self.sd["decoder.log_sigma"].data_ptr(), nll_bt.data_ptr(), B * T,
                         hp.input_nc * S * S)
            if loss_pre is None:
                la, kl_b = loss_args()
                plan.add("loss.kl", lib.gcpx_kl_gauss, *kl_args(kl_b, (B,)))
                plan.add("loss.combine", lib.gcpx_loss_combine, C.byref(la))
            else:
                la, kl_b = loss_pre
                plan.add("loss.final", lib.gcpx_loss_final, C.byref(la))
            loss_out = self._buf("losses", (16,), zero=True)
            outs["losses"], outs["nll_bt"], outs["kl_b"] = loss_out, nll_bt, kl_b
            outs["matched_distr_kernel_order"] = matched_distr

        outs.update(E=E, Hid=Hid, Z=Z, PZ=PZ, QZ=QZ, node_t=node_t, leave=leave, frame2node=f2n, seq_len=seq_len,
                    kept_idx=kept_idx, enc_traj_seq=enc_traj, inf_enc_seq=inf_enc, node2row=node2row, etilde_row=etrow)
        plan.rec.update(head_src=(prev if decode else None), tin=tin, key=key)
        if with_loss:
            plan.rec["loss_args"] = la
        plan.outs = outs
        return plan
```

### video-gcp_amd/plan_ops.py

```python
import ctypes as C
import os
from contextlib import contextmanager

import torch

from . import packing as pk
from . import runtime as rt
from .hparams import GCPHParams
from .params import init_params, encoder_layers, encoder_skip_layers, decoder_layers


def _addr(t, off_elems=0):
    return t.data_ptr() + 4 * off_elems


N_LANES = 3


class _Plan:

    def __init__(self, lib):
        self.lib = lib
        self.ops = []
        self.keep = []
        self.graph = None
        self.eager = False
        self.lane = 0
        self.rec = {}
        self.deferred = []
        self.tuned = None
        self.timed_ops = None
        self.split = None

    def add(self, name, fn, *args):
        self.ops.append((name, fn, args, self.lane))

    def _events(self, n):
        evs = []
        for _ in range(n):
            e = C.c_void_p()
            rt.check(self.lib.gcpx_event_create_sync(C.byref(e)), "event_create")
            evs.append(e)
        return evs

    def fork(self, lanes):
        self.ops.append(("@fork", None, (tuple(lanes), self._events(1)), 0))

    def join(self, lanes):
        self.ops.append(("@join", None, (tuple(lanes), self._events(len(lanes))), 0))

    def wait(self, waiter, signaler):
        self.ops.append(("@wait", None, (waiter, signaler, self._events(1)[0]), 0))

    def record(self, lane):
        ev = self._events(1)[0]
        self.ops.append(("@record", None, (lane, ev), 0))
        return ev

    def await_event(self, lane, ev):
        self.ops.append(("@await", None, (lane, ev), 0))

    def mark(self, tag, payload):
        self.ops.append(("@mark", None, (tag, payload), 0))

    def compact(self, streams, min_len=3, ranges=None):
        lib, out, run = self.lib, [], []
        inside = (lambda i: True) if ranges is None else (lambda i: any(a <= i < b for a, b in ranges))

        def flush():
            if len(run) >= min_len:
                st = streams[run[0][3]]
                rt.check(lib.gcpx_graph_begin(st), "graph_begin")
                for name, fn, args, _ in run:
                    rt.check(fn(*args, st), name)
                g = C.c_void_p()
                rt.check(lib.gcpx_graph_end(st, C.byref(g)), "graph_end")
                out.append(("@graph", None, (g, tuple(o[0] for o in run)), run[0][3]))
            else:
                out.extend(run)
            run.clear()
        for i, op in enumerate(self.ops):
            ctl = op[0].startswith("@") or not inside(i)
            if ctl or (run and op[3] != run[0][3]):
                flush()
            (out if ctl else run).append(op)
        flush()
        return out

    def run(self, streams, ops=None, on_mark=None):
        lib = self.lib
        for name, fn, args, lane in (self.ops if ops is None else ops):
            if name == "@mark":
                if on_mark is not None:
                    on_mark(*args)
            elif name == "@fork":
                lanes, evs = args
                rt.check(lib.gcpx_event_record(evs[0], streams[0]), "fork")
                for l in lanes:
                    rt.check(lib.gcpx_stream_wait_event(streams[l], evs[0]), "fork")
            elif name == "@wait":
                waiter, signaler, ev = args
                rt.check(lib.gcpx_event_record(ev, streams[signaler]), "wait")
                rt.check(lib.gcpx_stream_wait_event(streams[waiter], ev), "wait")
            elif name == "@graph":
                rt.check(lib.gcpx_graph_launch(args[0], streams[lane]), "graph_launch")
            elif name == "@record":
                rt.check(lib.gcpx_event_record(args[1], streams[args[0]]), "record")
            elif name == "@await":
                rt.check(lib.gcpx_stream_wait_event(streams[args[0]], args[1]), "await")
            elif name == "@join":
                lanes, evs = args
                for l, e in zip(lanes, evs):
                    rt.check(lib.gcpx_event_record(e, streams[l]), "join")
                    rt.check(lib.gcpx_stream_wait_event(streams[0], e), "join")
            else:
                st = fn(*args, streams[lane])
                if st != 0:
                    rt.check(st, name)


class Outputs(dict):
    __getattr__ = dict.__getitem__
    __setattr__ = dict.__setitem__


class ModelOutputs(Outputs):

    _LAZY = ("pruned_prediction", "actions", "regressed_state", "model_enc_seq", "cost", "cost_target")

    def __getattr__(self, name):
        if name in self:
            return self[name]
        if name in ModelOutputs._LAZY and "_model" in self:
            m = self["_model"]
            if name == "pruned_prediction":
                self[name] = m.pruned_prediction(self)
            else:
                aux = m.aux_outputs(self)
                for k in aux:
                    self.setdefault(k, aux[k])
            if name in self:
                return self[name]
        raise AttributeError(name)


class PlanOpsMixin:

    def _buf(self, name, shape, dtype=torch.float32, zero=False):
        key = (self._buf_prefix + name, tuple(shape), dtype)
        t = self._bufs.get(key)
        if t is None:
            t = (torch.zeros if zero else torch.empty)(tuple(shape), dtype=dtype, device=self.device)
            self._bufs[key] = t
        return t

    @staticmethod
    def _rowsrc(ptr, sb, sr, width, shift=0, rowidx=None, scale=None, shiftv=None, act=0, cmod=0):
        s = rt.RowSrc()
        s.ptr, s.rowidx = ptr, (rowidx.data_ptr() if rowidx is not None else None)
        s.scale = scale.data_ptr() if scale is not None else None
        s.shiftv = shiftv.data_ptr() if shiftv is not None else None
        s.sb, s.sr, s.width, s.shift, s.act, s.cmod = sb, sr, width, shift, act, cmod
        return s

    @staticmethod
    def _dense_rows(srcs, rpb, M):
        if rpb != 1 or M == 1 or any(s.shift != 0 for s in srcs):
            return srcs, rpb, False
        out = []
        for s in srcs:
            t = rt.RowSrc()
            t.ptr, t.rowidx, t.scale, t.shiftv = s.ptr, s.rowidx, s.scale, s.shiftv
            t.sb, t.sr = 0, (s.sr if s.rowidx else s.sb)
            t.width, t.shift, t.act, t.cmod = s.width, s.shift, s.act, s.cmod
            out.append(t)
        return out, M, True

    def _gemm_group(self, plan, name, group):
        if len(group) > 1:
            n = len(group)
            tab = (rt.GemmArgs * n)(*[a for _, a in group])
            dims = (C.c_int32 * (4 * n))()
            total = C.c_int32()
            if self.lib.gcpx_gemm_group_dims(tab, n, dims, C.byref(total)) == 0:
                raw = torch.frombuffer(bytearray(bytes(tab)), dtype=torch.uint8).to(self.device)
                dd = torch.tensor(list(dims), dtype=torch.int32, device=self.device)
                plan.keep += [raw, dd, tab]
                plan.add(name, self.lib.gcpx_gemm_group, raw.data_ptr(), dd.data_ptr(), n, total.value)
                return
        for nm, a in group:
            if a.epi == rt.EPI_GAUSS_SAMPLE:
                m, e = a.src[0], a.src[1]
                plan.add(nm, self.lib.gcpx_gauss_sample, m.ptr, m.sb, m.sr, e.ptr, e.sb, e.sr, a.out, a.ob, a.orow, a.M, a.rpb, a.N)
            else:
                plan.add(nm, self.lib.gcpx_gemm, C.byref(a))

    def _gemm(self, plan, name, srcs, M, N, rpb, wpk, bias, out=None, ob=0, orow=0, epi=rt.EPI_NONE,
              stats=None, lstm=None, batch=None, group=None, lstm_bwd=None):
        srcs, rpb, dense = self._dense_rows(srcs, rpb, M)
        if dense:
            ob, orow = 0, ob
            if lstm is not None:
                c_prev, c_prev_stride, h_out, c_out, hb, hrow, h_copy = lstm
                lstm = (c_prev, c_prev_stride, h_out, c_out, 0, hb, h_copy)
        a = rt.GemmArgs()
        for i, s in enumerate(srcs):
            a.src[i] = s
        a.nsrc, a.M, a.N, a.K, a.rpb = len(srcs), M, N, sum(s.width for s in srcs), rpb
        a.wpk, a.bias = wpk.data_ptr(), (bias.data_ptr() if bias is not None else None)
        gs = self._gsplit.get(wpk.data_ptr())
        if gs is not None and self.split_f16 and (self._arena is None or self._gsplit_live):
            a.wpk_split, a.w_split_log2_dev = gs[0].data_ptr(), gs[1].data_ptr()
        a.out, a.ob, a.orow, a.epi = out, ob, orow, epi
        a.stats_partial = stats.data_ptr() if stats is not None else None
        if lstm is not None:
            a.c_prev, a.c_prev_stride, a.h_out, a.c_out, a.hb, a.hrow, a.h_copy = lstm
            if self.save_for_backward:
                g = self._buf(f"gates.{name}", (M, N))
                a.gates_out = g.data_ptr()
                plan.rec[f"gates:{name}"] = g
        if batch is not None:
            a.nbatch, a.z_src_off, a.z_w_off, a.z_bias_off, a.z_out_off = batch
        if lstm_bwd is not None:
            a.lstm_bwd = lstm_bwd
        if a.wpk_split and M >= self._planes_min_rows and N >= 1024 and group is None and not a.stats_partial:
            nbytes, nexp = C.c_int64(), C.c_int64()
            rt.check(self.lib.gcpx_gemm_planes_workspace(M, a.K, a.nbatch, C.byref(nbytes), C.byref(nexp)), "planes workspace")
            wsb = self._buf(f"xplanes.l{plan.lane}", (nbytes.value,), torch.uint8)
            wse = self._buf(f"xexp.l{plan.lane}", (nexp.value,), torch.int32)
            a.x_planes, a.x_exp, a.x_planes_bytes = wsb.data_ptr(), wse.data_ptr(), nbytes.value
        plan.keep.append(a)
        if group is not None:
            group.append((name, a))
            return
        plan.add(name, self.lib.gcpx_gemm, C.byref(a))

    def _mlp(self, plan, name, W, srcs, M, rpb, out=None, ob=0, orow=0, oblk=0, out_split=0, gauss=None, group=None, tanh=False):
        hp = self._hp
        rec_srcs, rec_rpb = srcs, rpb
        srcs, rpb, dense = self._dense_rows(srcs, rpb, M)
        if dense:
            ob, orow = 0, ob
            if gauss is not None:
                eps, eb, erow, z, zb, zrow = gauss
                gauss = (eps, 0, eb, z, 0, zb)
        a = rt.MlpArgs()
        for i, s in enumerate(srcs):
            a.src[i] = s
        a.nsrc, a.M, a.rpb = len(srcs), M, rpb
        a.in_dim, a.mid, a.n_mid, a.out_dim = W["in_dim"], W["mid"], W["n_mid"], W["out_dim"]
        assert a.in_dim == sum(s.width for s in srcs), (name, a.in_dim)
        a.w_in, a.b_in = W["w_in"].data_ptr(), W["b_in"].data_ptr()
        if W["n_mid"]:
            a.w_mid, a.b_mid = W["w_mid"].data_ptr(), W["b_mid"].data_ptr()
            a.gn_gamma, a.gn_beta = W["gn_g"].data_ptr(), W["gn_b"].data_ptr()
        a.w_out, a.b_out = W["w_out"].data_ptr(), W["b_out"].data_ptr()
        a.gn_eps, a.lrelu_slope = hp.gn_eps, hp.leaky_slope
        a.out, a.ob, a.orow, a.oblk, a.out_split = out, ob, orow, oblk, out_split
        a.epi = rt.MLP_TANH if tanh else rt.MLP_PLAIN
        if gauss is not None:
            a.epi = rt.MLP_GAUSS
            a.eps, a.eb, a.erow, a.z, a.zb, a.zrow = gauss
        if self.save_for_backward:
            sv = self._buf(f"save.{name}", (1 + 2 * W["n_mid"], M, W["mid"]))
            a.save = sv.data_ptr()
            plan.rec[f"mlp:{name}"] = dict(W=W, srcs=rec_srcs, M=M, rpb=rec_rpb, save=sv)
        plan.keep.append(a)
        if group is not None:
            group.append((name, a))
            return
        plan.add(name, self.lib.gcpx_mlp, C.byref(a))

    def _mlp_group(self, plan, name, group, gemm=None):
        if len(group) == 1:
            if gemm is not None:
                plan.add(gemm[0], self.lib.gcpx_gemm, C.byref(gemm[1]))
            plan.add(group[0][0], self.lib.gcpx_mlp, C.byref(group[0][1]))
            return
        n = len(group)
        tab = (rt.MlpArgs * n)(*[a for _, a in group])
        dims = (C.c_int32 * (4 * n))()
        total = C.c_int32()
        rt.check(self.lib.gcpx_mlp_group_dims(tab, n, dims, C.byref(total)), name)
        raw = torch.frombuffer(bytearray(bytes(tab)), dtype=torch.uint8).to(self.device)
        dd = torch.tensor(list(dims), dtype=torch.int32, device=self.device)
        plan.keep += [raw, dd, tab]
        mid = group[0][1].mid
        if gemm is not None:
            if os.environ.get("GCPX_NO_LEVEL_PRE") is None and self.lib.gcpx_mlp_group_gemm_supported(C.byref(gemm[1]), total.value, mid):
                plan.add(f"{name}+{gemm[0]}", self.lib.gcpx_mlp_group_gemm, raw.data_ptr(), dd.data_ptr(), n, total.value, mid, C.byref(gemm[1]))
                return
            plan.add(gemm[0], self.lib.gcpx_gemm, C.byref(gemm[1]))
        plan.add(name, self.lib.gcpx_mlp_group, raw.data_ptr(), dd.data_ptr(), n, total.value, mid)

    def _bn(self, plan, tag, prefix, C_, stats, n_partial, pitch, count):
        sd, hp = self.sd, self._hp
        scale, shift = self._buf(f"{tag}.scale", (C_,)), self._buf(f"{tag}.shift", (C_,))
        g, b = sd[f"{prefix}.weight"], sd[f"{prefix}.bias"]
        if self.training:
            mean = rstd = None
            if self.save_for_backward:
                mean, rstd = self._buf(f"{tag}.mean", (C_,)), self._buf(f"{tag}.rstd", (C_,))
                plan.rec[f"bn:{tag}"] = dict(prefix=prefix, C=C_, count=count, scale=scale, shift=shift, mean=mean, rstd=rstd)
            plan.add(f"bn_finalize:{tag}", self.lib.gcpx_bn_finalize, stats.data_ptr(), n_partial, pitch, C_,
                     C.c_double(float(count)), g.data_ptr(), b.data_ptr(), C.c_float(hp.bn_eps), scale.data_ptr(),
                     shift.data_ptr(), None, None, C.c_float(0.0), rt.ptr(mean), rt.ptr(rstd))
        else:
            plan.add(f"bn_fold:{tag}", self.lib.gcpx_bn_fold, sd[f"{prefix}.running_mean"].data_ptr(),
                     sd[f"{prefix}.running_var"].data_ptr(), g.data_ptr(), b.data_ptr(), C.c_float(hp.bn_eps), C_,
                     scale.data_ptr(), shift.data_ptr())
        return scale, shift

    def _conv_args(self, srcs, F, Hin, Win, Hout, Wout, Cout, out_pitch, wpk, bias, out, upsample=0, out_act=0,
                   head_mode=rt.HEAD_RAW, images=None, stats=None):
        a = rt.ConvArgs()
        cin = 0
        for i, (t_ptr, C_, fdiv, scale, shift, act) in enumerate(srcs):
            s = a.src[i]
            s.ptr, s.C, s.frame_div, s.act = t_ptr, C_, fdiv, act
            s.scale = scale.data_ptr() if scale is not None else None
            s.shift = shift.data_ptr() if shift is not None else None
            cin += C_
        a.nsrc, a.F, a.Hin, a.Win, a.Hout, a.Wout, a.Cin, a.Cout = len(srcs), F, Hin, Win, Hout, Wout, cin, Cout
        a.out_pitch, a.upsample, a.out_act, a.head_mode = out_pitch, upsample, out_act, head_mode
        a.wpk, a.bias = wpk.data_ptr(), bias.data_ptr()
        a.out = out.data_ptr() if out is not None else None
        a.images = images.data_ptr() if images is not None else None
        a.stats_partial = stats.data_ptr() if stats is not None else None
        return a
```

Baseline: 476,100.

## Fuse split-f16 merge GEMM into level prior/posterior MLP group kernel

Moves the split-f16 GEMM body into a shared device tile header so it can be called from other kernels. Adds a combined level-pre kernel whose grid runs both the prior/posterior MLP row blocks and the 64x1 split-GEMM tiles of the next level's merge. The forward plan now folds wide merges into this single launch rather than forking them onto a side lane. The aim is to cut kernel launches and fill the GPU with both workloads at once. In exchange, the fused kernel must reserve the larger of the two LDS footprints, which may lower occupancy, and it gives up the side-stream overlap.

```diff
diff --git a/video-gcp_amd/csrc/gemm.hip b/video-gcp_amd/csrc/gemm.hip
--- a/video-gcp_amd/csrc/gemm.hip
+++ b/video-gcp_amd/csrc/gemm.hip
@@ -214,6 +214,11 @@
     return true;
 }
 
+bool gcpx_gemm_takes_split(const gcpx_gemm_args* a) {
+    int pr = 1, cr = 1;
+    return gemm_check(a) == GCPX_OK && !ks_block_choice(a, &pr, &cr) && !gcpx_gemm_planes_applies(a) && gcpx_gemm_split_applies(a);
+}
+
 extern "C" int gcpx_gemm(const gcpx_gemm_args* a, void* stream_) {
     hipStream_t stream = reinterpret_cast<hipStream_t>(stream_);
     const int st = gemm_check(a);
diff --git a/video-gcp_amd/csrc/gemm_split.hip b/video-gcp_amd/csrc/gemm_split.hip
--- a/video-gcp_amd/csrc/gemm_split.hip
+++ b/video-gcp_amd/csrc/gemm_split.hip
@@ -1,288 +1,15 @@
 #include "common.h"
+#include "gemm_split_tile.h"
 
 #include <cstdlib>
 #include <type_traits>
 
 namespace {
 
-typedef _Float16 h8 __attribute__((ext_vector_type(8)));
-typedef _Float16 h4 __attribute__((ext_vector_type(4)));
-typedef const f32x4 __attribute__((address_space(1)))* gptr4;
-__device__ __forceinline__ float4 gload4(const float* p) {
-    const f32x4 t = *(gptr4)p;
-    return make_float4(t[0], t[1], t[2], t[3]);
-}
-
-__device__ __forceinline__ f32x4 mfma32h(h8 a, h8 b, f32x4 c) {
-    return __builtin_amdgcn_mfma_f32_16x16x32_f16(a, b, c, 0, 0, 0);
-}
-
-template <int TN, int NSUB, int NW = 4>
-struct GsCfg {
-    static constexpr int TM = 16 * NW, THREADS = 64 * NW, KS = 32 * NSUB;
-    static constexpr int NCT = TN / 16;
-    static constexpr int W_SUB = NCT * 2048;
-    static constexpr int W_BYTES = NSUB * W_SUB;
-    static constexpr int X_SUB = NW * 2048;
-    static constexpr int X_BYTES = NSUB * X_SUB;
-    static constexpr int STAGE = W_BYTES + X_BYTES + 4 * TM;
-    static constexpr int LDS_BYTES = 2 * STAGE;
-    static constexpr int WLD = W_BYTES / (THREADS * 16);
-    static constexpr int WSTEP = THREADS * 16;
-};
-
 template <int TN, int NSUB, bool LSTM, bool XF, int NW = 4>
 __global__ void __launch_bounds__(64 * NW) gemm_split_kernel(const gcpx_gemm_args a) {
-    using Cfg = GsCfg<TN, NSUB, NW>;
-    constexpr int KS = Cfg::KS;
-    constexpr int NCT = Cfg::NCT, WLD = Cfg::WLD, CPW = NCT / 2;
     extern __shared__ float4 smem4[];
-    char* smem = reinterpret_cast<char*>(smem4);
-    const int tid = threadIdx.x, lane = tid & 63, wave = tid >> 6;
-    const int j = lane & 15, q = lane >> 4;
-    const int wr = wave >> 1, wc = wave & 1;
-    const int zb = blockIdx.z;
-    const int NT = a.N / 16;
-    const int ct0 = blockIdx.y * NCT;
-    const int M = a.M, rpb = a.rpb;
-    const int NK = a.K / KS;
-
-    const int srow = (wave << 4) + j, kq = q;
-    const int sr_ = blockIdx.x * Cfg::TM + srow;
-    const bool srv = sr_ < M;
-    const int srs = srv ? sr_ : 0;
-    const int srb = srs / rpb, srj = srs % rpb;
-    const int ew = a.w_split_log2_dev ? a.w_split_log2_dev[zb] : a.w_split_log2;
-    const int ex_cap = min(100, 126 - ew);
-    int ex_run = ex_cap;
-    int cur_s = -1, krem = 0, kloc = 0;
-    const float* xp = nullptr;
-    float xmask = 0.f;
-    const float* sp[6];
-    float sm[6];
-    int sw[6];
-#pragma unroll
-    for (int i = 0; i < 6; ++i) {
-        sp[i] = a.src[0].ptr; sm[i] = 0.f; sw[i] = 0;
-        if (i < a.nsrc) {
-            sw[i] = a.src[i].width / KS;
-            const gcpx_row_src& src = a.src[i];
-            bool ok = srv;
-            size_t off;
-            if (src.rowidx) {
-                off = (size_t)src.rowidx[srs] * src.sr;
-            } else {
-                const int jj = srj + src.shift;
-                ok = ok && jj >= 0 && jj < rpb;
-                off = (size_t)srb * src.sb + (size_t)(ok ? jj : 0) * src.sr;
-            }
-            sp[i] = src.ptr + (size_t)zb * a.z_src_off + off + kq * 8;
-            sm[i] = ok ? 1.f : 0.f;
-        }
-    }
-    auto next_source = [&]() {
-        ++cur_s;
-        xp = sp[0]; xmask = sm[0]; krem = sw[0];
-#pragma unroll
-        for (int i = 1; i < 6; ++i)
-            if (cur_s == i) { xp = sp[i]; xmask = sm[i]; krem = sw[i]; }
-        kloc = 0;
-    };
-    const char* wsrc = reinterpret_cast<const char*>(a.wpk_split) + (size_t)zb * a.z_w_off * 4 + (size_t)ct0 * 2048 + tid * 16;
-
-    struct RegSet {
-        float4 x[2 * NSUB], w[WLD];
-        float mask;
-        int src, k0;
-    };
-    RegSet rs[2];
-    const float* last_x = sp[0];
-    int last_s = 0;
-    auto issue = [&](const int s, RegSet& r) __attribute__((always_inline)) {
-        if (s < NK) {
-            if (krem == 0) next_source();
-            last_x = xp + kloc;
-            last_s = s;
-            r.mask = xmask; r.src = cur_s; r.k0 = kloc;
-            kloc += KS;
-            --krem;
-        }
-#pragma unroll
-        for (int h = 0; h < NSUB; ++h) {
-            r.x[2 * h] = gload4(last_x + 32 * h);
-            r.x[2 * h + 1] = gload4(last_x + 32 * h + 4);
-        }
-#pragma unroll
-        for (int i = 0; i < WLD; ++i) {
-            const int sub = i / (WLD / NSUB), c = i % (WLD / NSUB);
-            r.w[i] = *reinterpret_cast<const float4*>(wsrc + ((size_t)(NSUB * last_s + sub) * NT) * 2048 + c * Cfg::WSTEP);
-        }
-    };
-    auto commit = [&](const int st, RegSet& r) __attribute__((always_inline)) {
-        char* base = smem + st * Cfg::STAGE;
-#pragma unroll
-        for (int i = 0; i < WLD; ++i) {
-            const int sub = i / (WLD / NSUB), c = i % (WLD / NSUB);
-            *reinterpret_cast<float4*>(base + sub * Cfg::W_SUB + c * Cfg::WSTEP + tid * 16) = r.w[i];
-        }
-        if constexpr (XF) {
-#pragma unroll
-            for (int si = 0; si < 6; ++si) {
-                if (r.src == si && (a.src[si].scale || a.src[si].act)) {
-#pragma unroll
-                    for (int i = 0; i < 2 * NSUB; ++i)
-                        r.x[i] = affine_act4(r.x[i], a.src[si].scale, a.src[si].shiftv,
-                                             (r.k0 + 32 * (i >> 1) + 4 * (i & 1) + kq * 8) & (a.src[si].cmod - 1), a.src[si].act);
-                }
-            }
-        }
-        float amax = 0.f;
-#pragma unroll
-        for (int i = 0; i < 2 * NSUB; ++i) {
-            float4 v = r.x[i];
-            v.x *= r.mask; v.y *= r.mask; v.z *= r.mask; v.w *= r.mask;
-            r.x[i] = v;
-            amax = fmaxf(amax, fmaxf(fmaxf(fabsf(v.x), fabsf(v.y)), fmaxf(fabsf(v.z), fabsf(v.w))));
-        }
-        {
-            unsigned u = __float_as_uint(amax);
-            auto s16 = __builtin_amdgcn_permlane16_swap(u, u, false, false);
-            u = max(s16[0], s16[1]);
-            auto s32 = __builtin_amdgcn_permlane32_swap(u, u, false, false);
-            amax = __uint_as_float(max(s32[0], s32[1]));
-        }
-        if (amax > 0.f) {
-            const int ec = 14 + 127 - (int)((__float_as_uint(amax) >> 23) & 0xff);
-            ex_run = min(ex_run, max(-100, ec));
-        }
-        const float sc = __uint_as_float((unsigned)(127 + ex_run) << 23);
-        char* xb = base + Cfg::W_BYTES + (wave * 2) * 1024 + lane * 16;
-#pragma unroll
-        for (int h = 0; h < NSUB; ++h) {
-            const float4 v0 = r.x[2 * h], v1 = r.x[2 * h + 1];
-            const float f[8] = {v0.x * sc, v0.y * sc, v0.z * sc, v0.w * sc, v1.x * sc, v1.y * sc, v1.z * sc, v1.w * sc};
-            h8 p1, p2;
-#pragma unroll
-            for (int e = 0; e < 8; ++e) {
-                p1[e] = (_Float16)f[e];
-                p2[e] = (_Float16)fmaf((float)p1[e], -1.f, f[e]);
-            }
-            *reinterpret_cast<h8*>(xb + h * Cfg::X_SUB) = p1;
-            *reinterpret_cast<h8*>(xb + h * Cfg::X_SUB + 1024) = p2;
-        }
-        if (kq == 0) *reinterpret_cast<int*>(base + Cfg::W_BYTES + Cfg::X_BYTES + srow * 4) = ex_run;
-    };
-
-    f32x4 acc[CPW][2];
-#pragma unroll
-    for (int c = 0; c < CPW; ++c) { acc[c][0] = f32x4{0, 0, 0, 0}; acc[c][1] = f32x4{0, 0, 0, 0}; }
-    int excur[2] = {ex_cap, ex_cap};
-    auto compute = [&](const int st) __attribute__((always_inline)) {
-        const char* base = smem + st * Cfg::STAGE;
-        int en[2];
-#pragma unroll
-        for (int i = 0; i < 2; ++i) en[i] = *reinterpret_cast<const int*>(base + Cfg::W_BYTES + Cfg::X_BYTES + ((2 * wr + i) * 16 + j) * 4);
-        if (__any(en[0] != excur[0] || en[1] != excur[1])) {
-#pragma unroll
-            for (int i = 0; i < 2; ++i) {
-                const int d = en[i] - excur[i];
-                const float r = d < -126 ? 0.f : __uint_as_float((unsigned)(127 + d) << 23);
-#pragma unroll
-                for (int c = 0; c < CPW; ++c) acc[c][i] *= r;
-                excur[i] = en[i];
-            }
-        }
-#pragma unroll
-        for (int sub = 0; sub < NSUB; ++sub) {
-            h8 b[2][2];
-#pragma unroll
-            for (int i = 0; i < 2; ++i) {
-                const char* bp = base + Cfg::W_BYTES + sub * Cfg::X_SUB + ((2 * wr + i) * 2) * 1024 + lane * 16;
-                b[i][0] = *reinterpret_cast<const h8*>(bp);
-                b[i][1] = *reinterpret_cast<const h8*>(bp + 1024);
-            }
-            constexpr int CH = CPW <= 4 ? CPW : 2;
-#pragma unroll
-            for (int c0 = 0; c0 < CPW; c0 += CH) {
-                h8 w[CH][2];
-#pragma unroll
-                for (int c = 0; c < CH; ++c) {
-                    const char* wp = base + sub * Cfg::W_SUB + ((wc * CPW + c0 + c) * 2) * 1024 + lane * 16;
-                    w[c][0] = *reinterpret_cast<const h8*>(wp);
-                    w[c][1] = *reinterpret_cast<const h8*>(wp + 1024);
-                }
-#pragma unroll
-                for (int c = 0; c < CH; ++c)
-#pragma unroll
-                    for (int i = 0; i < 2; ++i) acc[c0 + c][i] = mfma32h(w[c][1], b[i][0], acc[c0 + c][i]);
-#pragma unroll
-                for (int c = 0; c < CH; ++c)
-#pragma unroll
-                    for (int i = 0; i < 2; ++i) acc[c0 + c][i] = mfma32h(w[c][0], b[i][1], acc[c0 + c][i]);
-#pragma unroll
-                for (int c = 0; c < CH; ++c)
-#pragma unroll
-                    for (int i = 0; i < 2; ++i) acc[c0 + c][i] = mfma32h(w[c][0], b[i][0], acc[c0 + c][i]);
-            }
-        }
-    };
-
-    issue(0, rs[0]);
-    issue(1, rs[1]);
-    commit(0, rs[0]);
-    issue(2, rs[0]);
-    __syncthreads();
-    for (int s = 0; s < NK; s += 2) {
-        compute(0);
-        __builtin_amdgcn_sched_barrier(0);
-        commit(1, rs[1]);
-        issue(s + 3, rs[1]);
-        __syncthreads();
-        if (s + 1 >= NK) break;
-        compute(1);
-        __builtin_amdgcn_sched_barrier(0);
-        commit(0, rs[0]);
-        issue(s + 4, rs[0]);
-        __syncthreads();
-    }
-
-#pragma unroll
-    for (int i = 0; i < 2; ++i) {
-        const int r = blockIdx.x * Cfg::TM + (2 * wr + i) * 16 + j;
-        const bool rv = r < M;
-        const int rs = rv ? r : 0;
-        const int rb = rs / rpb, rj = rs % rpb;
-        const float inv = __uint_as_float((unsigned)(127 - excur[i] - ew) << 23);
-#pragma unroll
-        for (int c = 0; c < CPW; ++c) {
-            const int nt = ct0 + wc * CPW + c;
-            const int n = nt * 16 + q * 4;
-            float4 bv = make_float4(0.f, 0.f, 0.f, 0.f);
-            if (a.bias) bv = *reinterpret_cast<const float4*>(a.bias + (size_t)zb * a.z_bias_off + n);
-            f32x4 v = acc[c][i];
-            v[0] = fmaf(v[0], inv, bv.x); v[1] = fmaf(v[1], inv, bv.y); v[2] = fmaf(v[2], inv, bv.z); v[3] = fmaf(v[3], inv, bv.w);
-            if (!rv) continue;
-            if constexpr (LSTM) {
-                const int u = nt * 4 + q;
-                const float cp = a.c_prev[(size_t)r * a.c_prev_stride + u];
-                const float ig = sigmoidf_(v[0]), fg = sigmoidf_(v[1]), gg = tanhf(v[2]), og = sigmoidf_(v[3]);
-                const float cn = fg * cp + ig * gg;
-                const float h = og * tanhf(cn);
-                const size_t o = (size_t)rb * a.hb + (size_t)rj * a.hrow + u;
-                a.h_out[o] = h;
-                a.c_out[o] = cn;
-                if (a.h_copy) a.h_copy[(size_t)r * (a.N / 4) + u] = h;
-                if (a.gates_out)
-                    *reinterpret_cast<float4*>(a.gates_out + ((size_t)r * (a.N / 4) + u) * 4) = make_float4(ig, fg, gg, og);
-            } else {
-                if (a.epi == GCPX_EPI_LRELU) {
-                    v[0] = lrelu(v[0], 0.2f); v[1] = lrelu(v[1], 0.2f); v[2] = lrelu(v[2], 0.2f); v[3] = lrelu(v[3], 0.2f);
-                }
-                float* op = a.out + (size_t)zb * a.z_out_off + (size_t)rb * a.ob + (size_t)rj * a.orow + n;
-                *reinterpret_cast<float4*>(op) = make_float4(v[0], v[1], v[2], v[3]);
-            }
-        }
-    }
+    gemm_split_tile<TN, NSUB, LSTM, XF, NW>(a, blockIdx.x, blockIdx.y, blockIdx.z, reinterpret_cast<char*>(smem4));
 }
 
 template <int TN, int NSUB, int NW = 4>
@@ -322,19 +49,32 @@
     return true;
 }
 
-int gcpx_launch_gemm_split(const gcpx_gemm_args* a, hipStream_t stream) {
+int gcpx_gemm_split_plan(const gcpx_gemm_args* a, int* gx, int* gy, int* gz) {
     const long nb = a->nbatch > 1 ? a->nbatch : 1;
     const long rbk = (a->M + 63) / 64;
     static const int force = [] { const char* e = getenv("GCPX_GEMM_SPLIT_CFG"); return e ? atoi(e) : 0; }();
-    if (force == 1282) return launch_split<128, 2>(a, stream);
-    if (force == 642) return launch_split<64, 2>(a, stream);
-    if (force == 641) return launch_split<64, 1>(a, stream);
-    if (force == 1281) return launch_split<128, 1>(a, stream);
-    if (force == 2561 && a->N % 256 == 0) return launch_split<256, 1>(a, stream);
-    if (force == 1288 && a->N % 128 == 0) return launch_split<128, 1, 8>(a, stream);
-    if (force == 2568 && a->N % 256 == 0) return launch_split<256, 1, 8>(a, stream);
-    if (a->N % 256 == 0 && ((a->M + 127) / 128) * (long)(a->N / 256) * nb >= 256) return launch_split<256, 1, 8>(a, stream);
-    if (a->N % 128 == 0 && ((a->M + 127) / 128) * (long)(a->N / 128) * nb >= 512) return launch_split<128, 1, 8>(a, stream);
-    if (a->N % 128 == 0 && rbk * (a->N / 128) * nb >= 768) return launch_split<128, 1>(a, stream);
-    return launch_split<64, 1>(a, stream);
+    int cfg = 641;
+    if (force == 1282 || force == 642 || force == 641 || force == 1281) cfg = force;
+    else if (force == 2561 && a->N % 256 == 0) cfg = force;
+    else if (force == 1288 && a->N % 128 == 0) cfg = force;
+    else if (force == 2568 && a->N % 256 == 0) cfg = force;
+    else if (a->N % 256 == 0 && ((a->M + 127) / 128) * (long)(a->N / 256) * nb >= 256) cfg = 2568;
+    else if (a->N % 128 == 0 && ((a->M + 127) / 128) * (long)(a->N / 128) * nb >= 512) cfg = 1288;
+    else if (a->N % 128 == 0 && rbk * (a->N / 128) * nb >= 768) cfg = 1281;
+    const int tm = cfg % 10 == 8 ? 128 : 64;
+    *gx = (a->M + tm - 1) / tm; *gy = a->N / (cfg / 10); *gz = (int)nb;
+    return cfg;
 }
+
+int gcpx_launch_gemm_split(const gcpx_gemm_args* a, hipStream_t stream) {
+    int gx, gy, gz;
+    switch (gcpx_gemm_split_plan(a, &gx, &gy, &gz)) {
+        case 1282: return launch_split<128, 2>(a, stream);
+        case 642: return launch_split<64, 2>(a, stream);
+        case 1281: return launch_split<128, 1>(a, stream);
+        case 2561: return launch_split<256, 1>(a, stream);
+        case 1288: return launch_split<128, 1, 8>(a, stream);
+        case 2568: return launch_split<256, 1, 8>(a, stream);
+        default: return launch_split<64, 1>(a, stream);
+    }
+}
diff --git a/video-gcp_amd/csrc/gemm_split_tile.h b/video-gcp_amd/csrc/gemm_split_tile.h
--- /dev/null
+++ b/video-gcp_amd/csrc/gemm_split_tile.h
@@ -0,0 +1,286 @@
+#pragma once
+#include "common.h"
+
+#include <type_traits>
+
+namespace {
+
+typedef _Float16 h8 __attribute__((ext_vector_type(8)));
+typedef _Float16 h4 __attribute__((ext_vector_type(4)));
+typedef const f32x4 __attribute__((address_space(1)))* gptr4;
+__device__ __forceinline__ float4 gload4(const float* p) {
+    const f32x4 t = *(gptr4)p;
+    return make_float4(t[0], t[1], t[2], t[3]);
+}
+
+__device__ __forceinline__ f32x4 mfma32h(h8 a, h8 b, f32x4 c) {
+    return __builtin_amdgcn_mfma_f32_16x16x32_f16(a, b, c, 0, 0, 0);
+}
+
+template <int TN, int NSUB, int NW = 4>
+struct GsCfg {
+    static constexpr int TM = 16 * NW, THREADS = 64 * NW, KS = 32 * NSUB;
+    static constexpr int NCT = TN / 16;
+    static constexpr int W_SUB = NCT * 2048;
+    static constexpr int W_BYTES = NSUB * W_SUB;
+    static constexpr int X_SUB = NW * 2048;
+    static constexpr int X_BYTES = NSUB * X_SUB;
+    static constexpr int STAGE = W_BYTES + X_BYTES + 4 * TM;
+    static constexpr int LDS_BYTES = 2 * STAGE;
+    static constexpr int WLD = W_BYTES / (THREADS * 16);
+    static constexpr int WSTEP = THREADS * 16;
+};
+
+template <int TN, int NSUB, bool LSTM, bool XF, int NW = 4>
+__device__ __forceinline__ void gemm_split_tile(const gcpx_gemm_args& a, const int bx, const int by, const int bz, char* smem) {
+    using Cfg = GsCfg<TN, NSUB, NW>;
+    constexpr int KS = Cfg::KS;
+    constexpr int NCT = Cfg::NCT, WLD = Cfg::WLD, CPW = NCT / 2;
+    const int tid = threadIdx.x, lane = tid & 63, wave = tid >> 6;
+    const int j = lane & 15, q = lane >> 4;
+    const int wr = wave >> 1, wc = wave & 1;
+    const int zb = bz;
+    const int NT = a.N / 16;
+    const int ct0 = by * NCT;
+    const int M = a.M, rpb = a.rpb;
+    const int NK = a.K / KS;
+
+    const int srow = (wave << 4) + j, kq = q;
+    const int sr_ = bx * Cfg::TM + srow;
+    const bool srv = sr_ < M;
+    const int srs = srv ? sr_ : 0;
+    const int srb = srs / rpb, srj = srs % rpb;
+    const int ew = a.w_split_log2_dev ? a.w_split_log2_dev[zb] : a.w_split_log2;
+    const int ex_cap = min(100, 126 - ew);
+    int ex_run = ex_cap;
+    int cur_s = -1, krem = 0, kloc = 0;
+    const float* xp = nullptr;
+    float xmask = 0.f;
+    const float* sp[6];
+    float sm[6];
+    int sw[6];
+#pragma unroll
+    for (int i = 0; i < 6; ++i) {
+        sp[i] = a.src[0].ptr; sm[i] = 0.f; sw[i] = 0;
+        if (i < a.nsrc) {
+            sw[i] = a.src[i].width / KS;
+            const gcpx_row_src& src = a.src[i];
+            bool ok = srv;
+            size_t off;
+            if (src.rowidx) {
+                off = (size_t)src.rowidx[srs] * src.sr;
+            } else {
+                const int jj = srj + src.shift;
+                ok = ok && jj >= 0 && jj < rpb;
+                off = (size_t)srb * src.sb + (size_t)(ok ? jj : 0) * src.sr;
+            }
+            sp[i] = src.ptr + (size_t)zb * a.z_src_off + off + kq * 8;
+            sm[i] = ok ? 1.f : 0.f;
+        }
+    }
+    auto next_source = [&]() {
+        ++cur_s;
+        xp = sp[0]; xmask = sm[0]; krem = sw[0];
+#pragma unroll
+        for (int i = 1; i < 6; ++i)
+            if (cur_s == i) { xp = sp[i]; xmask = sm[i]; krem = sw[i]; }
+        kloc = 0;
+    };
+    const char* wsrc = reinterpret_cast<const char*>(a.wpk_split) + (size_t)zb * a.z_w_off * 4 + (size_t)ct0 * 2048 + tid * 16;
+
+    struct RegSet {
+        float4 x[2 * NSUB], w[WLD];
+        float mask;
+        int src, k0;
+    };
+    RegSet rs[2];
+    const float* last_x = sp[0];
+    int last_s = 0;
+    auto issue = [&](const int s, RegSet& r) __attribute__((always_inline)) {
+        if (s < NK) {
+            if (krem == 0) next_source();
+            last_x = xp + kloc;
+            last_s = s;
+            r.mask = xmask; r.src = cur_s; r.k0 = kloc;
+            kloc += KS;
+            --krem;
+        }
+#pragma unroll
+        for (int h = 0; h < NSUB; ++h) {
+            r.x[2 * h] = gload4(last_x + 32 * h);
+            r.x[2 * h + 1] = gload4(last_x + 32 * h + 4);
+        }
+#pragma unroll
+        for (int i = 0; i < WLD; ++i) {
+            const int sub = i / (WLD / NSUB), c = i % (WLD / NSUB);
+            r.w[i] = *reinterpret_cast<const float4*>(wsrc + ((size_t)(NSUB * last_s + sub) * NT) * 2048 + c * Cfg::WSTEP);
+        }
+    };
+    auto commit = [&](const int st, RegSet& r) __attribute__((always_inline)) {
+        char* base = smem + st * Cfg::STAGE;
+#pragma unroll
+        for (int i = 0; i < WLD; ++i) {
+            const int sub = i / (WLD / NSUB), c = i % (WLD / NSUB);
+            *reinterpret_cast<float4*>(base + sub * Cfg::W_SUB + c * Cfg::WSTEP + tid * 16) = r.w[i];
+        }
+        if constexpr (XF) {
+#pragma unroll
+            for (int si = 0; si < 6; ++si) {
+                if (r.src == si && (a.src[si].scale || a.src[si].act)) {
+#pragma unroll
+                    for (int i = 0; i < 2 * NSUB; ++i)
+                        r.x[i] = affine_act4(r.x[i], a.src[si].scale, a.src[si].shiftv,
+                                             (r.k0 + 32 * (i >> 1) + 4 * (i & 1) + kq * 8) & (a.src[si].cmod - 1), a.src[si].act);
+                }
+            }
+        }
+        float amax = 0.f;
+#pragma unroll
+        for (int i = 0; i < 2 * NSUB; ++i) {
+            float4 v = r.x[i];
+            v.x *= r.mask; v.y *= r.mask; v.z *= r.mask; v.w *= r.mask;
+            r.x[i] = v;
+            amax = fmaxf(amax, fmaxf(fmaxf(fabsf(v.x), fabsf(v.y)), fmaxf(fabsf(v.z), fabsf(v.w))));
+        }
+        {
+            unsigned u = __float_as_uint(amax);
+            auto s16 = __builtin_amdgcn_permlane16_swap(u, u, false, false);
+            u = max(s16[0], s16[1]);
+            auto s32 = __builtin_amdgcn_permlane32_swap(u, u, false, false);
+            amax = __uint_as_float(max(s32[0], s32[1]));
+        }
+        if (amax > 0.f) {
+            const int ec = 14 + 127 - (int)((__float_as_uint(amax) >> 23) & 0xff);
+            ex_run = min(ex_run, max(-100, ec));
+        }
+        const float sc = __uint_as_float((unsigned)(127 + ex_run) << 23);
+        char* xb = base + Cfg::W_BYTES + (wave * 2) * 1024 + lane * 16;
+#pragma unroll
+        for (int h = 0; h < NSUB; ++h) {
+            const float4 v0 = r.x[2 * h], v1 = r.x[2 * h + 1];
+            const float f[8] = {v0.x * sc, v0.y * sc, v0.z * sc, v0.w * sc, v1.x * sc, v1.y * sc, v1.z * sc, v1.w * sc};
+            h8 p1, p2;
+#pragma unroll
+            for (int e = 0; e < 8; ++e) {
+                p1[e] = (_Float16)f[e];
+                p2[e] = (_Float16)fmaf((float)p1[e], -1.f, f[e]);
+            }
+            *reinterpret_cast<h8*>(xb + h * Cfg::X_SUB) = p1;
+            *reinterpret_cast<h8*>(xb + h * Cfg::X_SUB + 1024) = p2;
+        }
+        if (kq == 0) *reinterpret_cast<int*>(base + Cfg::W_BYTES + Cfg::X_BYTES + srow * 4) = ex_run;
+    };
+
+    f32x4 acc[CPW][2];
+#pragma unroll
+    for (int c = 0; c < CPW; ++c) { acc[c][0] = f32x4{0, 0, 0, 0}; acc[c][1] = f32x4{0, 0, 0, 0}; }
+    int excur[2] = {ex_cap, ex_cap};
+    auto compute = [&](const int st) __attribute__((always_inline)) {
+        const char* base = smem + st * Cfg::STAGE;
+        int en[2];
+#pragma unroll
+        for (int i = 0; i < 2; ++i) en[i] = *reinterpret_cast<const int*>(base + Cfg::W_BYTES + Cfg::X_BYTES + ((2 * wr + i) * 16 + j) * 4);
+        if (__any(en[0] != excur[0] || en[1] != excur[1])) {
+#pragma unroll
+            for (int i = 0; i < 2; ++i) {
+                const int d = en[i] - excur[i];
+                const float r = d < -126 ? 0.f : __uint_as_float((unsigned)(127 + d) << 23);
+#pragma unroll
+                for (int c = 0; c < CPW; ++c) acc[c][i] *= r;
+                excur[i] = en[i];
+            }
+        }
+#pragma unroll
+        for (int sub = 0; sub < NSUB; ++sub) {
+            h8 b[2][2];
+#pragma unroll
+            for (int i = 0; i < 2; ++i) {
+                const char* bp = base + Cfg::W_BYTES + sub * Cfg::X_SUB + ((2 * wr + i) * 2) * 1024 + lane * 16;
+                b[i][0] = *reinterpret_cast<const h8*>(bp);
+                b[i][1] = *reinterpret_cast<const h8*>(bp + 1024);
+            }
+            constexpr int CH = CPW <= 4 ? CPW : 2;
+#pragma unroll
+            for (int c0 = 0; c0 < CPW; c0 += CH) {
+                h8 w[CH][2];
+#pragma unroll
+                for (int c = 0; c < CH; ++c) {
+                    const char* wp = base + sub * Cfg::W_SUB + ((wc * CPW + c0 + c) * 2) * 1024 + lane * 16;
+                    w[c][0] = *reinterpret_cast<const h8*>(wp);
+                    w[c][1] = *reinterpret_cast<const h8*>(wp + 1024);
+                }
+#pragma unroll
+                for (int c = 0; c < CH; ++c)
+#pragma unroll
+                    for (int i = 0; i < 2; ++i) acc[c0 + c][i] = mfma32h(w[c][1], b[i][0], acc[c0 + c][i]);
+#pragma unroll
+                for (int c = 0; c < CH; ++c)
+#pragma unroll
+                    for (int i = 0; i < 2; ++i) acc[c0 + c][i] = mfma32h(w[c][0], b[i][1], acc[c0 + c][i]);
+#pragma unroll
+                for (int c = 0; c < CH; ++c)
+#pragma unroll
+                    for (int i = 0; i < 2; ++i) acc[c0 + c][i] = mfma32h(w[c][0], b[i][0], acc[c0 + c][i]);
+            }
+        }
+    };
+
+    issue(0, rs[0]);
+    issue(1, rs[1]);
+    commit(0, rs[0]);
+    issue(2, rs[0]);
+    __syncthreads();
+    for (int s = 0; s < NK; s += 2) {
+        compute(0);
+        __builtin_amdgcn_sched_barrier(0);
+        commit(1, rs[1]);
+        issue(s + 3, rs[1]);
+        __syncthreads();
+        if (s + 1 >= NK) break;
+        compute(1);
+        __builtin_amdgcn_sched_barrier(0);
+        commit(0, rs[0]);
+        issue(s + 4, rs[0]);
+        __syncthreads();
+    }
+
+#pragma unroll
+    for (int i = 0; i < 2; ++i) {
+        const int r = bx * Cfg::TM + (2 * wr + i) * 16 + j;
+        const bool rv = r < M;
+        const int rs = rv ? r : 0;
+        const int rb = rs / rpb, rj = rs % rpb;
+        const float inv = __uint_as_float((unsigned)(127 - excur[i] - ew) << 23);
+#pragma unroll
+        for (int c = 0; c < CPW; ++c) {
+            const int nt = ct0 + wc * CPW + c;
+            const int n = nt * 16 + q * 4;
+            float4 bv = make_float4(0.f, 0.f, 0.f, 0.f);
+            if (a.bias) bv = *reinterpret_cast<const float4*>(a.bias + (size_t)zb * a.z_bias_off + n);
+            f32x4 v = acc[c][i];
+            v[0] = fmaf(v[0], inv, bv.x); v[1] = fmaf(v[1], inv, bv.y); v[2] = fmaf(v[2], inv, bv.z); v[3] = fmaf(v[3], inv, bv.w);
+            if (!rv) continue;
+            if constexpr (LSTM) {
+                const int u = nt * 4 + q;
+                const float cp = a.c_prev[(size_t)r * a.c_prev_stride + u];
+                const float ig = sigmoidf_(v[0]), fg = sigmoidf_(v[1]), gg = tanhf(v[2]), og = sigmoidf_(v[3]);
+                const float cn = fg * cp + ig * gg;
+                const float h = og * tanhf(cn);
+                const size_t o = (size_t)rb * a.hb + (size_t)rj * a.hrow + u;
+                a.h_out[o] = h;
+                a.c_out[o] = cn;
+                if (a.h_copy) a.h_copy[(size_t)r * (a.N / 4) + u] = h;
+                if (a.gates_out)
+                    *reinterpret_cast<float4*>(a.gates_out + ((size_t)r * (a.N / 4) + u) * 4) = make_float4(ig, fg, gg, og);
+            } else {
+                if (a.epi == GCPX_EPI_LRELU) {
+                    v[0] = lrelu(v[0], 0.2f); v[1] = lrelu(v[1], 0.2f); v[2] = lrelu(v[2], 0.2f); v[3] = lrelu(v[3], 0.2f);
+                }
+                float* op = a.out + (size_t)zb * a.z_out_off + (size_t)rb * a.ob + (size_t)rj * a.orow + n;
+                *reinterpret_cast<float4*>(op) = make_float4(v[0], v[1], v[2], v[3]);
+            }
+        }
+    }
+}
+
+}
diff --git a/video-gcp_amd/csrc/mlp.hip b/video-gcp_amd/csrc/mlp.hip
--- a/video-gcp_amd/csrc/mlp.hip
+++ b/video-gcp_amd/csrc/mlp.hip
@@ -1,9 +1,12 @@
 #include "common.h"
 #include "gemm_tile.h"
+#include "gemm_split_tile.h"
 
 #include <cstdlib>
 
 bool gcpx_gemm_tile_plan(const gcpx_gemm_args* a, int* pr, int* cr, int* ks, int* gx, int* gy, int* gz);
+bool gcpx_gemm_takes_split(const gcpx_gemm_args* a);
+int gcpx_gemm_split_plan(const gcpx_gemm_args* a, int* gx, int* gy, int* gz);
 
 namespace {
 
@@ -335,6 +338,32 @@
     return nullptr;
 }
 
+using LpsCfg = GsCfg<64, 1, 4>;
+constexpr int LPS_HID_BYTES = 2 * 16 * (128 + 4) * 4;
+constexpr int LPS_LDS_BYTES = LpsCfg::LDS_BYTES > LPS_HID_BYTES ? LpsCfg::LDS_BYTES : LPS_HID_BYTES;
+__global__ void __launch_bounds__(256) level_pre_split_kernel(const gcpx_mlp_args* __restrict__ tab, const int4* __restrict__ dims, const int n,
+                                                              const int nblocks, const gcpx_gemm_args g, const int gx, const int gy) {
+    extern __shared__ float4 lps_smem4[];
+    const int blk = blockIdx.x;
+    if (blk >= nblocks) {
+        const int local = blk - nblocks;
+        gemm_split_tile<64, 1, false, false, 4>(g, local % gx, (local / gx) % gy, local / (gx * gy), reinterpret_cast<char*>(lps_smem4));
+        return;
+    }
+    int p = 0;
+    while (p + 1 < n && blk >= dims[p + 1].x) ++p;
+    const int4 d = dims[p];
+    const int local = blk - d.x;
+    mlp_rows<128, true>(tab[p], local % d.y, local / d.y, d.z, reinterpret_cast<float*>(lps_smem4));
+}
+
+bool level_pre_split_applies(const gcpx_gemm_args* g, int* gx, int* gy, int* gz) {
+    if (!gcpx_gemm_takes_split(g)) return false;
+    for (int s = 0; s < g->nsrc; ++s)
+        if (g->src[s].scale || g->src[s].act) return false;
+    return gcpx_gemm_split_plan(g, gx, gy, gz) == 641;
+}
+
 int mlp_check(const gcpx_mlp_args* a) {
     GCPX_CHECK_ARG(a != nullptr, "null args");
     GCPX_CHECK_ARG(a->nsrc >= 1 && a->nsrc <= 6, "nsrc out of range");
@@ -413,6 +442,10 @@
 
 extern "C" int gcpx_mlp_group_gemm_supported(const gcpx_gemm_args* g, int32_t total_blocks, int32_t mid) {
     if (!g || mid != 128 || g->epi == GCPX_EPI_LSTM || g->epi == GCPX_EPI_GAUSS_SAMPLE) return 0;
+    {
+        int gx, gy, gz;
+        if (level_pre_split_applies(g, &gx, &gy, &gz)) return 1;
+    }
     const int cus = gcpx_conv_grid() / 2;
     if (total_blocks > cus) return 0;
     int pr, cr, ks, gx, gy, gz;
@@ -426,6 +459,22 @@
     GCPX_CHECK_ARG(dev_table && dev_dims && g && n >= 1 && n <= 16 && total_blocks > 0, "bad arguments");
     GCPX_CHECK_ARG((((uintptr_t)dev_dims) & 15) == 0, "dims must be 16-byte aligned");
     int pr, cr, ks, gx, gy, gz;
+    if (mid == 128 && g->epi != GCPX_EPI_LSTM && g->epi != GCPX_EPI_GAUSS_SAMPLE && level_pre_split_applies(g, &gx, &gy, &gz)) {
+        static bool attr_set = false;
+        if (!attr_set) {
+            hipError_t e = hipFuncSetAttribute(reinterpret_cast<const void*>(level_pre_split_kernel), hipFuncAttributeMaxDynamicSharedMemorySize,
+                                               LPS_LDS_BYTES);
+            if (e != hipSuccess) {
+                gcpx_set_error("gcpx_mlp_group_gemm: hipFuncSetAttribute(%d B LDS): %s", LPS_LDS_BYTES, hipGetErrorString(e));
+                return GCPX_ERR_HIP;
+            }
+            attr_set = true;
+        }
+        hipLaunchKernelGGL(level_pre_split_kernel, dim3(total_blocks + gx * gy * gz), dim3(256), LPS_LDS_BYTES, stream, dev_table,
+                           reinterpret_cast<const int4*>(dev_dims), n, total_blocks, *g, gx, gy);
+        GCPX_CHECK_LAUNCH();
+        return GCPX_OK;
+    }
     level_pre_fn kern = nullptr;
     if (mid == 128 && g->epi != GCPX_EPI_LSTM && g->epi != GCPX_EPI_GAUSS_SAMPLE && gcpx_gemm_tile_plan(g, &pr, &cr, &ks, &gx, &gy, &gz))
         kern = level_pre_variant(pr, cr, ks);
diff --git a/video-gcp_amd/forward_plan.py b/video-gcp_amd/forward_plan.py
--- a/video-gcp_amd/forward_plan.py
+++ b/video-gcp_amd/forward_plan.py
@@ -269,6 +269,7 @@
             plan_bookkeeping()
 
         side_merge = False
+        wide_merge = []
         for l in range(L):
             W = P[f"tree{l if hp.untied_layers else 0}"]
             s = 2 ** (L - 1 - l)
@@ -319,8 +320,9 @@
                 g = (_addr(tin["eps"], (n - 1) * nv), N * nv, nv) + z_map
                 self._mlp(plan, f"posterior{l}", W["q"], [el(), er(), et], M, n, out=_addr(QZ, nodeoff(2 * nv)),
                           ob=PS * 2 * nv, orow=2 * s * 2 * nv, gauss=g, group=pq)
-                mg = []
-                if l > 0 and merge_with_predictors and not side_merge:
+                mg = wide_merge
+                wide_merge = []
+                if l > 0 and merge_with_predictors and not side_merge and not mg:
                     plan_merge(l, group=mg)
                 self._mlp_group(plan, f"prior+posterior{l}", pq, gemm=(mg[0] if mg else None))
                 if side_merge:
@@ -364,11 +366,18 @@
                 plan_merge(l + 1, group=g)
             self._gemm_group(plan, f"out{l}+merge{l + 1}" if len(g) > 1 else f"out{l}", g)
             if (l + 1 < L and merge_with_predictors and hp.tree_lstm == "split_linear" and B * 2 ** (l + 1) >= self._merge_side_rows):
-                plan.fork([1])
-                plan.lane = 1
-                plan_merge(l + 1)
-                plan.lane = 0
-                side_merge = True
+                probe = []
+                plan_merge(l + 1, group=probe)
+                pa = probe[0][1]
+                planes = pa.wpk_split and pa.M >= self._planes_min_rows and pa.N >= 1024
+                if not planes and self._level_pre_ok(pa, 1 << 24, W["prior"]["mid"]):
+                    wide_merge = probe
+                else:
+                    plan.fork([1])
+                    plan.lane = 1
+                    plan_merge(l + 1)
+                    plan.lane = 0
+                    side_merge = True
 
         F = B * N
         matching = adaptive and has_traj and phase == "train"
diff --git a/video-gcp_amd/plan_ops.py b/video-gcp_amd/plan_ops.py
--- a/video-gcp_amd/plan_ops.py
+++ b/video-gcp_amd/plan_ops.py
@@ -271,6 +271,9 @@
             return
         plan.add(name, self.lib.gcpx_mlp, C.byref(a))
 
+    def _level_pre_ok(self, gemm_args, total_blocks, mid):
+        return os.environ.get("GCPX_NO_LEVEL_PRE") is None and bool(self.lib.gcpx_mlp_group_gemm_supported(C.byref(gemm_args), total_blocks, mid))
+
     def _mlp_group(self, plan, name, group, gemm=None):
         if len(group) == 1:
             if gemm is not None:
@@ -287,7 +290,7 @@
         plan.keep += [raw, dd, tab]
         mid = group[0][1].mid
         if gemm is not None:
-            if os.environ.get("GCPX_NO_LEVEL_PRE") is None and self.lib.gcpx_mlp_group_gemm_supported(C.byref(gemm[1]), total.value, mid):
+            if self._level_pre_ok(gemm[1], total.value, mid):
                 plan.add(f"{name}+{gemm[0]}", self.lib.gcpx_mlp_group_gemm, raw.data_ptr(), dd.data_ptr(), n, total.value, mid, C.byref(gemm[1]))
                 return
             plan.add(gemm[0], self.lib.gcpx_gemm, C.byref(gemm[1]))
```

After: 478,800 (median of 6 runs). Within noise of the previous version (+0.6%).
